# xp3i4/linear

Measured on AMD Instinct MI355X. Metric: reads/sec (whole node) + HBM GB/s on seed lookup, 10 kb reads vs GRCh38, higher is better.
Workload: dtype u64

## Files before the change

linear_amd/build.py:

```python
from __future__ import annotations

import os
import shutil
import subprocess

HERE = os.path.dirname(os.path.abspath(__file__))
CSRC = os.path.join(HERE, "csrc")
SO = os.path.join(HERE, "liblinear_amd.so")
CLI = os.path.join(HERE, "linear_filter")
SOURCES = sorted(f for f in os.listdir(CSRC) if f.endswith((".hip", ".h", ".cpp", ".inc")))
FLAGS = ["--offload-arch=gfx950", "-O3", "-std=c++17", "-ffp-contract=off", "-fPIC", "-shared"]


def hipcc_path() -> str:
    for c in (shutil.which("hipcc"), "/opt/rocm/bin/hipcc"):
        if c and os.path.exists(c):
            return c
    raise RuntimeError("hipcc not found: the MI355X library cannot be built")


def needs_build() -> bool:
    if not os.path.exists(SO) or not os.path.exists(CLI):
        return True
    t = os.path.getmtime(SO)
    deps = [os.path.join(CSRC, s) for s in SOURCES] + [os.path.join(HERE, "..", "include", "linear_amd.h")]
    return any(os.path.getmtime(d) > t for d in deps)


DEVICE_TUS = ["lnr_api.hip", "lnr_gap_kernels.hip", "lnr_output_kernels.hip", "lnr_reader_kernels.hip"]
OUT_GPU = {"lnr_output_kernels.hip", "lnr_output_hd.h", "lnr_output_hook.h", "lnr_deflate_hd.h", "lnr_inflate_hd.h"}
RD_GPU = {"lnr_reader_kernels.hip", "lnr_reader_hd.h", "lnr_reader_hook.h", "lnr_inflate_hd.h", "lnr_bam_hd.h"}
API_HOST = {"lnr_host_util.h", "lnr_ctx.h", "lnr_index.h", "lnr_batch.h", "lnr_gap_stage.h"}
NOT_A_DEP = {"lnr_api.hip": {"lnr_gap_kernels.hip", "lnr_gap_hd.h", "lnr_reader.cpp", "lnr_output.cpp", "linear_filter_main.cpp"} | OUT_GPU | RD_GPU,
             "lnr_gap_kernels.hip": {"lnr_api.hip", "lnr_kernels.hip", "lnr_reader.cpp", "lnr_output.cpp", "linear_filter_main.cpp"} | OUT_GPU | RD_GPU | API_HOST,
             "lnr_output_kernels.hip": set(SOURCES) - OUT_GPU - {"ref_sort.h"},
             "lnr_reader_kernels.hip": set(SOURCES) - RD_GPU,
             "lnr_reader.cpp": set(SOURCES) - {"lnr_reader.cpp", "lnr_reader_hook.h", "lnr_inflate_hd.h", "lnr_bam_hd.h"}, "lnr_output.cpp": set(SOURCES) - {"lnr_output.cpp", "lnr_output_hook.h"}}


def stale(obj: str, src: str) -> bool:
    if not os.path.exists(obj):
        return True
    t = os.path.getmtime(obj)
    deps = [os.path.join(CSRC, f) for f in SOURCES if f not in NOT_A_DEP[src]] + [os.path.join(HERE, "..", "include", "linear_amd.h"), os.path.abspath(__file__)]
    return any(os.path.getmtime(d) > t for d in deps)


def build(force: bool = False, defines: tuple = (), out: str | None = None, only: tuple | None = None) -> str:
    so = out or SO
    if out and only:
        build()
        tag = "." + os.path.basename(out).replace(".so", "")
        stock = [os.path.join(HERE, s.replace(".cpp", ".o")) for s in ("lnr_reader.cpp", "lnr_output.cpp")] + [os.path.join(HERE, s.replace(".hip", ".o")) for s in DEVICE_TUS if s not in only]
        mine = [(os.path.join(HERE, s.replace(".hip", tag + ".o")), s) for s in only]
        note, want = out + ".defines", " ".join(defines) + "\n"
        same = os.path.exists(note) and open(note).read() == want
        if not force and same and os.path.exists(out) and not any(stale(o, s) or os.path.getmtime(o) > os.path.getmtime(out) for o, s in mine) and all(os.path.getmtime(o) <= os.path.getmtime(out) for o in stock):
            return out
        for obj, src in mine:
            cmd = [hipcc_path()] + [f for f in FLAGS if f != "-shared"] + list(defines) + ["-c", os.path.join(CSRC, src), "-o", obj]
            if subprocess.call(cmd):
                raise RuntimeError("compile failed: " + " ".join(cmd))
        os.makedirs(os.path.dirname(out), exist_ok=True)
        subprocess.check_call([hipcc_path(), "--offload-arch=gfx950", "-fPIC", "-shared", "-o", out] + ["-Wl," + o for o in stock + [o for o, _ in mine]] + ["-lz", "-lpthread"])
        with open(note, "w") as f:
            f.write(want)
        return out
    if force or out or needs_build():
        from concurrent.futures import ThreadPoolExecutor
        tag = "" if not out else "." + os.path.basename(out).replace(".so", "")
        jobs = []
        for src in ("lnr_reader.cpp", "lnr_output.cpp"):
            obj = os.path.join(HERE, src.replace(".cpp", ".o"))
            jobs.append((obj, None if not (force or stale(obj, src)) else ["g++", "-O2", "-std=c++17", "-fPIC", "-Wall", "-Wextra", "-c", os.path.join(CSRC, src), "-o", obj]))
        for src in DEVICE_TUS:
            obj = os.path.join(HERE, src.replace(".hip", tag + ".o"))
            jobs.append((obj, None if not (force or out or stale(obj, src)) else
                         [hipcc_path()] + [f for f in FLAGS if f != "-shared"] + list(defines) + ["-c", os.path.join(CSRC, src), "-o", obj]))
        with ThreadPoolExecutor(len(jobs)) as ex:
            for rc, (obj, cmd) in zip(ex.map(lambda j: subprocess.call(j[1]) if j[1] else 0, jobs), jobs):
                if rc:
                    raise RuntimeError("compile failed: " + " ".join(cmd))
        objs = ["-Wl," + o for o, _ in jobs]
        subprocess.check_call([hipcc_path(), "--offload-arch=gfx950", "-fPIC", "-shared", "-o", so] + objs + ["-lz", "-lpthread"])
        if not out:
            subprocess.check_call(["g++", "-O2", "-std=c++17", "-Wall", "-Wextra", os.path.join(CSRC, "linear_filter_main.cpp"), "-o", CLI, SO,
                                   "-Wl,-rpath,$ORIGIN", "-Wl,-rpath,/opt/rocm/lib", "-L/opt/rocm/lib", "-lpthread"])
    return so


VARIANT_DIR = os.path.join(HERE, "..", "tools", "_variants")
GAP_VARIANTS = {
    "columns": ("-DK_GAP_COL_MIN=64", "-DK_GAP_COL_MEAN=1", "-DK_GAP_YB_MIN=64", "-DK_GAP_SORT_TEAM_MIN=128", "-DK_GAP_JOIN_TEAM_MIN=256"),
    "scan": ("-DK_GAP_COL_MIN=64", "-DK_GAP_COL_MEAN=1", "-DK_GAP_YB_MIN=1000000000", "-DK_GAP_SORT_TEAM_MIN=128", "-DK_GAP_JOIN_TEAM_MIN=256"),
    "rows": ("-DK_GAP_COL_MIN=1000000000", "-DK_GAP_TEAM_ROW=256", "-DK_GAP_SINGLE_MAX=1024", "-DK_GAP_SORT_TEAM_MIN=128", "-DK_GAP_JOIN_TEAM_MIN=256"),
}


def gap_variant_path(name: str) -> str:
    return os.path.abspath(os.path.join(VARIANT_DIR, "gap_" + name + ".so"))


def build_gap_variants() -> list:
    from concurrent.futures import ThreadPoolExecutor
    build()
    with ThreadPoolExecutor(len(GAP_VARIANTS)) as ex:
        return list(ex.map(lambda kv: build(defines=kv[1], out=gap_variant_path(kv[0]), only=("lnr_gap_kernels.hip",)), GAP_VARIANTS.items()))


if __name__ == "__main__":
    import sys
    if len(sys.argv) > 1:
        vdir = os.path.join(HERE, "..", "tools", "_variants")
        os.makedirs(vdir, exist_ok=True)
        print(build(defines=tuple(sys.argv[2:]), out=os.path.join(vdir, sys.argv[1] + ".so")))
    else:
        print(build(force=True))
```

linear_amd/csrc/lnr_api.hip:

```cpp
#include <cstring>
#include <rocprim/device/device_radix_sort.hpp>
#include "lnr_kernels.hip"
#include "lnr_gap_args.h"
#include "../../include/linear_amd.h"

#include <algorithm>
#include <dlfcn.h>
#include <chrono>
#include <cstdio>
#include <cstdlib>
#include <atomic>
#include <condition_variable>
#include <deque>
#include <memory>
#include <mutex>
#include <string>
#include <thread>
#include <vector>

using namespace lnr;

#include "lnr_host_util.h"
#include "lnr_ctx.h"
#include "lnr_index.h"
#include "lnr_batch.h"

namespace {

lnr_status submit_reads(lnr_ctx *ctx, Lane *L, int slot, const u8 *reads, const u64 *off, u32 n) {
    if (!off || (n && !reads)) { ctx->err = "null read buffer"; return LNR_ERR_ARG; }
    for (u32 i = 0; i < n; i++)
        if (off[i + 1] < off[i]) { ctx->err = "read offsets not monotone"; return LNR_ERR_ARG; }
    u64 base = off[0], total = off[n] - off[0];
    DevBuf &dr = L->in_reads[slot], &dof = L->in_off[slot];
    AllocCount count_(&L->allocs);
    ENSURE(dr, std::max<u64>(total, 16));
    ENSURE(dof, ((size_t)n + 1) * 8);
    if (!L->h_off[slot].ensure(((size_t)n + 1) * 8)) { ctx->err = "pinned host allocation failed"; return LNR_ERR_NOMEM; }
    u64 *o = L->h_off[slot].as<u64>();
    for (u32 i = 0; i <= n; i++) o[i] = off[i] - base;
    hipStream_t sc = ctx->s_copy;
    if (total) {
        hipPointerAttribute_t at;
        bool pinned = hipPointerGetAttributes(&at, reads + base) == hipSuccess && at.type == hipMemoryTypeHost;
        if (!pinned) (void)hipGetLastError();
        if (pinned) {
            HIPCK(hipMemcpyAsync(dr.p, reads + base, total, hipMemcpyHostToDevice, sc));
        } else {
            const u64 CH = 32ULL << 20;
            for (int k = 0; k < 2; k++) {
                if (!ctx->h_up[k].ensure(CH)) { ctx->err = "pinned host allocation failed"; return LNR_ERR_NOMEM; }
                HIPCK(ctx->ev_up[k].create());
            }
            int k = 0;
            for (u64 o2 = 0; o2 < total; o2 += CH, k ^= 1) {
                u64 len = std::min<u64>(CH, total - o2);
                HIPCK(hipEventSynchronize(ctx->ev_up[k]));
                par_memcpy(ctx->h_up[k].p, reads + base + o2, len);
                HIPCK(hipMemcpyAsync(dr.as<u8>() + o2, ctx->h_up[k].p, len, hipMemcpyHostToDevice, sc));
                HIPCK(hipEventRecord(ctx->ev_up[k], sc));
            }
        }
    }
    HIPCK(hipMemcpyAsync(dof.p, o, ((size_t)n + 1) * 8, hipMemcpyHostToDevice, sc));
    HIPCK(hipEventRecord(L->ev_in[slot], sc));
    L->in_n[slot] = n;
    return LNR_OK;
}

std::unique_ptr<Lane> lane_create(lnr_ctx *ctx, int id) {
    std::unique_ptr<Lane> L(new (std::nothrow) Lane());
    if (!L) return nullptr;
    L->opts = &ctx->opts; L->tun = &ctx->tun; L->ix = &ctx->ix; L->id = id;
    if (!L->init(id == 1 ? ctx->tun.lane1_prio : 0)) return nullptr;
    return L;
}

void lane_release_batch(Lane *L) {
    for (int k = 0; k < 2; k++) { L->js[k].anchors.release(); L->js[k].cap_slots = 0; }
    L->ln.job_scr.release(); L->tb_remap.scr.release(); L->tb_early.scr.release(); L->tb_late.scr.release();
    L->pk.release(); L->nm.release(); L->f1.release(); L->cords.release(); L->out_str.release(); L->out_end.release(); L->gaps.release(); L->gdense.release();
}

lnr_status compute_slot(Lane *C, Lane *In, int slot, Pre &P) {
    P = Pre();
    P.valid = true; P.tot = 0; P.n = In->in_n[slot];
    hipError_t e = hipStreamWaitEvent(C->stream, In->ev_in[slot], 0);
    P.st = e == hipSuccess ? filter_dev(C, In->in_reads[slot].as<u8>(), In->in_off[slot].as<u64>(), In->in_n[slot], nullptr, In->h_off[slot].as<u64>()) : LNR_ERR_HIP;
    P.err = C->err.get();
    P.stats = C->stats;
    if (P.st == LNR_OK) {
        P.tot = C->last_ncords;
        if (C->h_cord_off.size() != (size_t)P.n + 1) C->h_cord_off.assign((size_t)P.n + 1, 0);
        P.coff = C->h_cord_off;
        P.d_str = C->r_str.p; P.d_end = C->r_end.p;
    }
    return P.st;
}
lnr_status compute_submitted(lnr_ctx *ctx) {
    int slot = ctx->in_head;
    ctx->in_head = (ctx->in_head + 1) % 3; ctx->in_count--;
    return compute_slot(ctx->lane[0].get(), ctx->lane[0].get(), slot, ctx->pre);
}

void lane_worker(lnr_ctx *top, int li) {
    Lane &Ln = *top->lane[li], &L0 = *top->lane[0];
    (void)hipSetDevice(top->device);
    std::unique_lock<std::mutex> lk(top->mu);
    auto take_set = [](Lane &R, Ticket *T) {
        T->res_set = R.set_used[0] ? 1 : 0;
        R.set_used[T->res_set] = true;
    };
    auto run = [&](Lane &R, Ticket *T) {
        if (T->res_set != R.set_cur) { R.r_off.swap(R.rB_off); R.r_str.swap(R.rB_str); R.r_end.swap(R.rB_end); R.set_cur = T->res_set; }
        compute_slot(&R, &Ln, T->slot, T->pre);
        if (T->pre.st == LNR_OK && !R.rB_str.p) {
            AllocCount count_(&R.allocs);
            (void)R.rB_off.ensure(R.r_off.cap); (void)R.rB_off.host_stage(R.r_off.hcap); (void)R.rB_str.ensure(R.r_str.cap); (void)R.rB_end.ensure(R.r_end.cap);
        }
    };
    for (;;) {
        top->cv.wait(lk, [&] { return top->quit || (!Ln.work.empty() && (li == 1 || (Ln.unhanded < 2 && !Ln.busy && !(top->lane1_off && top->lane[1] && top->lane[1]->pending > 0))) && (li == 0 || top->lane1_off || Ln.unhanded < 2)); });
        if (top->quit) return;
        Ticket *T = Ln.work.front();
        Ln.work.pop_front();
        bool on_own = li == 0 || !top->lane1_off;
        if (on_own) {
            Ln.busy = true;
            take_set(Ln, T);
            lk.unlock();
            if (li == 1 && top->lane1_nomem_test) { top->lane1_nomem_test = false; T->pre = Pre(); T->pre.valid = true; T->pre.st = LNR_ERR_NOMEM; T->pre.err = "LNR_LANE1_NOMEM: allocation failure injected"; }
            else run(Ln, T);
            lk.lock();
            Ln.busy = false;
            if (li == 1 && T->pre.st == LNR_ERR_NOMEM) {
                Ln.set_used[T->res_set] = false;
                top->lane1_off = true;
                on_own = false;
                lk.unlock();
                Ln.sync();
                lane_release_batch(&Ln);
                if (getenv("LNR_DEBUG_TIMES")) fprintf(stderr, "[lnr] lane 1 out of memory: its batch runs again on lane 0, one lane from now on\n");
                lk.lock();
                top->cv.notify_all();
            }
        }
        if (!on_own) {
            top->cv.wait(lk, [&] { return top->quit || (!L0.busy && L0.unhanded < 2); });
            if (top->quit) return;
            L0.busy = true;
            take_set(L0, T);
            lk.unlock();
            run(L0, T);
            lk.lock();
            L0.busy = false;
        }
        Lane &R = on_own ? Ln : L0;
        T->res_lane = on_own ? li : 0;
        T->done = true;
        Ln.slot_busy[T->slot] = false; Ln.pending--; R.unhanded++;
        top->cv.notify_all();
    }
}

lnr_status hand_out(lnr_ctx *ctx, u32 n, u64 tot, std::vector<u64> &&coff, const void *d_str, const void *d_end, hipStream_t st, hipStream_t after, lnr_cords *out) {
    const int rs = ctx->res_slot;
    ctx->res_slot ^= 1;
    PinBuf &hs_ = ctx->h_cords_str2[rs], &he_ = ctx->h_cords_end2[rs];
    if (!hs_.ensure(std::max<u64>(tot * 8, 16)) || !he_.ensure(std::max<u64>(tot * 8, 16))) { ctx->err = "pinned host allocation failed"; return LNR_ERR_NOMEM; }
    ctx->h_cord_off2[rs] = std::move(coff);
    if (tot) {
        if (after) { HIPCK(hipEventRecord(ctx->ev_done, after)); HIPCK(hipStreamWaitEvent(st, ctx->ev_done, 0)); }
        HIPCK(hipMemcpyAsync(hs_.p, d_str, tot * 8, hipMemcpyDeviceToHost, st));
        HIPCK(hipMemcpyAsync(he_.p, d_end, tot * 8, hipMemcpyDeviceToHost, st));
    }
    out->n_reads = n; out->n_cords = tot;
    out->cord_off = ctx->h_cord_off2[rs].data(); out->cords_str = hs_.as<u64>(); out->cords_end = he_.as<u64>();
    return LNR_OK;
}

lnr_status lane0_result(lnr_ctx *ctx, lnr_status st) {
    if (st != LNR_OK) ctx->err = ctx->lane[0]->err.get();
    ctx->stats_pub = ctx->lane[0]->stats;
    return st;
}

}

extern "C" {

void lnr_opts_default(lnr_opts *o) {
    if (!o) return;
    memset(o, 0, sizeof *o);
    o->device = -1; o->index_type = 1; o->feature_type = 2; o->preset = 1; o->gap_len = 0; o->dup = 0; o->scratch_budget = 0;
}

const char *lnr_strerror(lnr_status s) {
    switch (s) {
        case LNR_OK: return "ok";
        case LNR_ERR_ARG: return "invalid argument";
        case LNR_ERR_NO_DEVICE: return "no usable HIP device (this library has no CPU path)";
        case LNR_ERR_HIP: return "HIP runtime error";
        case LNR_ERR_NOMEM: return "out of memory";
        case LNR_ERR_NO_INDEX: return "index not built";
        case LNR_ERR_LIMIT: return "input exceeds a format limit";
        case LNR_ERR_UNSUPPORTED: return "option not supported by this build";
        case LNR_ERR_INTERNAL: return "internal capacity overflow";
    }
    return "unknown status";
}
const char *lnr_last_error(const lnr_ctx *ctx) { return ctx ? const_cast<lnr_ctx *>(ctx)->err.show() : "null context"; }

lnr_status lnr_create(const lnr_opts *opts, lnr_ctx **out) {
    if (!out) return LNR_ERR_ARG;
    *out = nullptr;
    lnr_opts o;
    if (opts) o = *opts; else lnr_opts_default(&o);
    if ((o.index_type != 1 && o.index_type != 2) || o.feature_type != 2 || (o.preset != 1 && o.preset != 2) || o.dup > 1) return LNR_ERR_UNSUPPORTED;
    int ndev = 0;
    if (hipGetDeviceCount(&ndev) != hipSuccess || ndev <= 0) { (void)hipGetLastError(); return LNR_ERR_NO_DEVICE; }
    int dev = o.device;
    if (dev < 0) { if (hipGetDevice(&dev) != hipSuccess) return LNR_ERR_NO_DEVICE; }
    if (dev >= ndev) return LNR_ERR_ARG;
    int prev_dev = -1;
    (void)hipGetDevice(&prev_dev);
    if (hipSetDevice(dev) != hipSuccess) return LNR_ERR_NO_DEVICE;
    struct Restore { int d; ~Restore() { if (d >= 0) (void)hipSetDevice(d); } } restore_{prev_dev == dev ? -1 : prev_dev};
    lnr_ctx *ctx = new (std::nothrow) lnr_ctx();
    if (!ctx) return LNR_ERR_NOMEM;
    ctx->opts = o;
    ctx->device = dev;
    ctx->tun = tuning_from_env(dev);
    ctx->lane1_nomem_test = ctx->tun.lane1_nomem;
    ctx->lane[0] = lane_create(ctx, 0);
    bool ok = ctx->lane[0] && ctx->s_copy.create() && ctx->s_down.create() && ctx->ev_down.create() == hipSuccess && ctx->ev_done.create() == hipSuccess;
    if (!ok) { (void)hipGetLastError(); lnr_destroy(ctx); return LNR_ERR_HIP; }
    *out = ctx;
    return LNR_OK;
}

void lnr_destroy(lnr_ctx *ctx) {
    if (!ctx) return;
    (void)hipSetDevice(ctx->device);
    { std::lock_guard<std::mutex> g(ctx->mu); ctx->quit = true; }
    ctx->cv.notify_all();
    for (auto &L : ctx->lane) if (L && L->th.joinable()) L->th.join();
    ctx->s_copy.sync(); ctx->s_down.sync();
    delete ctx;
}

lnr_status lnr_filter_batch_dev(lnr_ctx *ctx, const uint8_t *d_reads, const uint64_t *d_off, uint32_t n, lnr_cords_dev *out) {
    if (!ctx || !d_off || (n && !d_reads)) return LNR_ERR_ARG;
    DevGuard dg_(ctx->device);
    if (in_flight(ctx)) { ctx->err = "batches submitted with lnr_filter_submit are still in flight"; return LNR_ERR_ARG; }
    return lane0_result(ctx, filter_dev(ctx->lane[0].get(), d_reads, d_off, n, out));
}
lnr_status lnr_last_gaps(lnr_ctx *ctx, lnr_gaps *out) {
    if (!ctx || !out) return LNR_ERR_ARG;
    DevGuard dg_(ctx->device);
    if (!ctx->tickets.empty()) { ctx->err = "lnr_last_gaps: batches are in flight (a worker is writing the per-read arrays)"; return LNR_ERR_ARG; }
    Lane *L = ctx->lane[0].get();
    u32 n = L->last_n;
    out->n_reads = n; out->n_gaps = 0; out->gap_off = nullptr; out->gaps = nullptr;
    ctx->h_gap_off.assign((size_t)n + 1, 0);
    ctx->h_gap_pairs.clear();
    if (n && L->last_gaps_off.size() == n) {
        std::vector<u32> ng(n);
        HIPCK(hipStreamSynchronize(L->stream));
        HIPCK(hipMemcpy(ng.data(), L->ngaps.p, (size_t)n * 4, hipMemcpyDeviceToHost));
        for (u32 i = 0; i < n; i++) ctx->h_gap_off[i + 1] = ctx->h_gap_off[i] + ng[i];
        ctx->h_gap_pairs.resize(2 * ctx->h_gap_off[n]);
        u64 last = L->last_gaps_off[n - 1];
        std::vector<UP> all;
        {
            u64 total_cap = last + 4 + (1u << 10);
            if (total_cap * sizeof(UP) > L->gaps.cap) total_cap = L->gaps.cap / sizeof(UP);
            all.resize(total_cap);
            if (total_cap) HIPCK(hipMemcpy(all.data(), L->gaps.p, total_cap * sizeof(UP), hipMemcpyDeviceToHost));
        }
        for (u32 i = 0; i < n; i++)
            for (u32 k = 0; k < ng[i]; k++) {
                const UP &g = all[L->last_gaps_off[i] + k];
                ctx->h_gap_pairs[2 * (ctx->h_gap_off[i] + k)] = g.first; ctx->h_gap_pairs[2 * (ctx->h_gap_off[i] + k) + 1] = g.second;
            }
    }
    out->n_gaps = ctx->h_gap_off[n];
    out->gap_off = ctx->h_gap_off.data(); out->gaps = ctx->h_gap_pairs.data();
    return LNR_OK;
}
lnr_status lnr_cords_to_host(lnr_ctx *ctx, lnr_cords *out) {
    if (!ctx || !out) return LNR_ERR_ARG;
    DevGuard dg_(ctx->device);
    if (!ctx->tickets.empty()) { ctx->err = "lnr_cords_to_host: batches are in flight"; return LNR_ERR_ARG; }
    Lane *L = ctx->lane[0].get();
    u64 tot = L->last_ncords;
    if (L->h_cord_off.size() != (size_t)L->last_n + 1) L->h_cord_off.assign((size_t)L->last_n + 1, 0);
    lnr_status s = hand_out(ctx, L->last_n, tot, std::vector<u64>(L->h_cord_off), L->r_str.p, L->r_end.p, L->stream, nullptr, out);
    if (s != LNR_OK) return s;
    if (tot) HIPCK(hipStreamSynchronize(L->stream));
    return LNR_OK;
}
void *lnr_host_alloc(size_t bytes) {
    void *p = nullptr;
    if (hipHostMalloc(&p, bytes ? bytes : 16, hipHostMallocDefault) != hipSuccess) { (void)hipGetLastError(); return nullptr; }
    return p;
}
void lnr_host_free(void *p) { if (p) (void)hipHostFree(p); }

lnr_status lnr_filter_submit(lnr_ctx *ctx, const uint8_t *reads, const uint64_t *off, uint32_t n) {
    if (!ctx) return LNR_ERR_ARG;
    DevGuard dg_(ctx->device);
    if (!ctx->ix.has_index) { ctx->err = "no index"; return LNR_ERR_NO_INDEX; }
    if (ctx->in_count + (ctx->pre.valid ? 1 : 0) + ctx->tickets.size() >= 3) { ctx->err = "three batches already in flight: call lnr_filter_wait first"; return LNR_ERR_ARG; }
    if (two_lanes(ctx)) {
        int li = (ctx->tickets.empty() || ctx->lane1_off) ? 0 : (ctx->tickets.back()->lane ^ 1);
        if (li == 1 && !ctx->lane[1]) {
            std::unique_ptr<Lane> L1 = lane_create(ctx, 1);
            if (L1) { std::lock_guard<std::mutex> g(ctx->mu); ctx->lane[1] = std::move(L1); }
            else { ctx->lane1_off = true; li = 0; }
        }
        int slot = 0;
        for (;;) {
            Lane &Ln = *ctx->lane[li];
            { std::lock_guard<std::mutex> g(ctx->mu); slot = 0; while (slot < 2 && Ln.slot_busy[slot]) slot++; }
            lnr_status s = submit_reads(ctx, &Ln, slot, reads, off, n);
            if (s == LNR_ERR_NOMEM && li == 1) { ctx->lane1_off = true; li = 0; continue; }
            if (s != LNR_OK) return s;
            break;
        }
        Lane &Ln = *ctx->lane[li];
        if (!Ln.th.joinable()) {
            try { Ln.th = std::thread(lane_worker, ctx, li); }
            catch (...) { ctx->err = "worker thread could not be started"; return LNR_ERR_INTERNAL; }
        }
        std::unique_ptr<Ticket> T(new Ticket());
        T->lane = li; T->slot = slot;
        {
            std::lock_guard<std::mutex> g(ctx->mu);
            Ln.slot_busy[slot] = true; Ln.pending++;
            Ln.work.push_back(T.get());
        }
        ctx->tickets.push_back(std::move(T));
        ctx->cv.notify_all();
        return LNR_OK;
    }
    int slot = (ctx->in_head + ctx->in_count) % 3;
    lnr_status s = submit_reads(ctx, ctx->lane[0].get(), slot, reads, off, n);
    if (s != LNR_OK) return s;
    ctx->in_count++;
    return LNR_OK;
}
lnr_status lnr_filter_wait(lnr_ctx *ctx, lnr_cords *out) {
    if (!ctx || !out) return LNR_ERR_ARG;
    DevGuard dg_(ctx->device);
    if (!ctx->tickets.empty()) {
        Ticket *T = ctx->tickets.front().get();
        { std::unique_lock<std::mutex> lk(ctx->mu); ctx->cv.wait(lk, [&] { return T->done; }); }
        Pre P = std::move(T->pre);
        Lane &Ln = *ctx->lane[T->res_lane];
        const int T_set = T->res_set;
        ctx->tickets.pop_front();
        struct Free { lnr_ctx *c; Lane &l; int set; ~Free() { { std::lock_guard<std::mutex> g(c->mu); l.unhanded--; l.set_used[set] = false; } c->cv.notify_all(); } } free_{ctx, Ln, T_set};
        if (P.st != LNR_OK) { ctx->err = P.err; return P.st; }
        lnr_status s = hand_out(ctx, P.n, P.tot, std::move(P.coff), P.d_str, P.d_end, ctx->s_down, nullptr, out);
        if (s != LNR_OK) return s;
        if (P.tot) HIPCK(hipStreamSynchronize(ctx->s_down));
        ctx->stats_pub = P.stats;
        return LNR_OK;
    }
    if (!ctx->pre.valid) {
        if (ctx->in_count == 0) { ctx->err = "no batch in flight"; return LNR_ERR_ARG; }
        compute_submitted(ctx);
    }
    Pre P = std::move(ctx->pre);
    ctx->pre = Pre();
    if (P.st != LNR_OK) { ctx->err = P.err; return P.st; }
// ... 83 lines not shown
```

linear_amd/csrc/lnr_batch.h:

```cpp
#pragma once
#include "lnr_gap_stage.h"

namespace {

struct HostJobs {
    std::vector<u32> read, str, end, mode, grp_beg;
    u64 nsamp = 0;
    void add(u32 r, u32 s, u32 e, u32 m) {
        read.push_back(r); str.push_back(s); end.push_back(e); mode.push_back(m);
        nsamp += seed_num_samples(s, e, (u32)job_parm((int)m).alpha);
    }
    u32 size() const { return (u32)read.size(); }
};

struct BatchHost {
    u32 n = 0;
    std::vector<u64> off;
    std::vector<u32> len, nf, cords_cap, gaps_cap;
    std::vector<u64> f1_off, cords_off, gaps_off, pk_off;
};

JobArrays job_arrays(JobSet &S) {
    JobArrays J;
    J.read = S.j_read.as<u32>(); J.str = S.j_str.as<u32>(); J.end = S.j_end.as<u32>(); J.mode = S.j_mode.as<u32>();
    return J;
}
ReadArrays read_arrays(Lane *L) {
    ReadArrays R;
    R.len = L->rlen.as<u32>(); R.ks = L->rks.as<i32>();
    R.pk = L->pk.as<u64>(); R.nm = L->nm.as<u32>(); R.pk_off = L->pk_off.as<u64>();
    return R;
}

lnr_status launch_f1(Lane *L, u32 n) {
    LCK(hipEventRecord(L->ev_prep, L->stream));
    LCK(hipStreamWaitEvent(L->s_bulk, L->ev_prep, 0));
    hipLaunchKernelGGL(k_f1, dim3(n), dim3(256), 0, L->s_bulk, L->pk.as<u64>(), L->nm.as<u32>(), L->pk_off.as<u64>(), L->rlen.as<u32>(), L->nf.as<u32>(), L->f1_off.as<u64>(), n,
                       L->f1.as<F96>()); LKCHECK();
    LCK(hipEventRecord(L->ev_f1, L->s_bulk));
    return LNR_OK;
}

lnr_status seed_jobs(Lane *L, JobSet &S, const HostJobs &hj, hipStream_t st, u32 f1_reads = 0) {
    const Index &ix = *L->ix; const Tuning &tun = *L->tun;
    u32 nj = hj.size();
    S.cap.assign(nj, 0); S.look.assign(nj, 0); S.nanc.assign(nj, 0); S.anc_off.assign(nj, 0);
    if (nj == 0) return f1_reads ? launch_f1(L, f1_reads) : LNR_OK;
    lnr_status s;
    if ((s = upload_on(L->err, S.j_read, hj.read, st)) != LNR_OK) return s;
    if ((s = upload_on(L->err, S.j_str, hj.str, st)) != LNR_OK) return s;
    if ((s = upload_on(L->err, S.j_end, hj.end, st)) != LNR_OK) return s;
    if ((s = upload_on(L->err, S.j_mode, hj.mode, st)) != LNR_OK) return s;
    if ((s = upload_on(L->err, S.grp_beg, hj.grp_beg, st)) != LNR_OK) return s;
    LENSURE(S.j_cap, (size_t)nj * 4);
    LENSURE(S.j_look, (size_t)nj * 4);
    LENSURE(S.j_nanc, (size_t)nj * 4);
    LENSURE(S.j_anc_off, (size_t)nj * 8);
    LENSURE(S.seed_ctl, 64);
    if (!S.t_seed.a) S.t_seed.init();
    JobArrays J = job_arrays(S);
    ReadArrays R = read_arrays(L);
    u64 first_segs = ((hj.nsamp * S.est_x16) >> 4) + (u64)nj * 194;
    u64 need_slots = first_segs * 2 + (1u << 20);
    if (need_slots > S.cap_slots) S.cap_slots = need_slots + need_slots / 2;
    u64 anc_slots = S.cap_slots;
    bool use_bm = tun.seed_bm < 0 ? ix.info.hs_len < (1ULL << 25) : tun.seed_bm != 0;
    for (int attempt = 0; ; attempt++) {
        LENSURE(S.anchors, anc_slots * 8);
        LCK(hipMemsetAsync(S.seed_ctl.p, 0, 64, st));
        SeedOutArrays O;
        O.cursor = S.seed_ctl.as<unsigned long long>(); O.overflow = (int *)(S.seed_ctl.as<char>() + 16); O.capacity = anc_slots;
        O.anchors = S.anchors.as<u64>(); O.anc_off = S.j_anc_off.as<u64>(); O.job_cap = S.j_cap.as<u32>(); O.job_look = S.j_look.as<u32>();
        O.n_anchors = S.j_nanc.as<u32>();
        S.t_seed.start(st);
        if (L->opts->index_type == 2)
            hipLaunchKernelGGL(k_seed_hindex, dim3(nj), dim3(64), 0, st, J, R, ix.hs.as<u64>(), ix.info.hs_len, ix.hx_empty_dir, ix.dir.as<i32>(), ix.hx_nkeys.as<u64>(), ix.hx_nvals.as<u32>(), ix.hx_nnodes, nj, O,
                               S.est_x16);
        else
        hipLaunchKernelGGL(k_seed_fused, dim3(nj), dim3(64), tun.seed_lds_pad, st, J, R, ix.bl.as<ulonglong2>(), use_bm ? ix.bm.as<u32>() : (const u32 *)nullptr, ix.ov.as<u64>(), nj, O, S.est_x16); LKCHECK();
        S.t_seed.stop(st);
        if (f1_reads && attempt == 0) { lnr_status fs = launch_f1(L, f1_reads); if (fs != LNR_OK) return fs; }
        int ovf = 0;
        Readback rb;
        if (!rb.begin(S.h_rb, (size_t)nj * 20 + 256)) { L->err = "pinned host allocation failed"; return LNR_ERR_NOMEM; }
        LCK(rb.add(S.cap.data(), S.j_cap.p, (size_t)nj * 4, st));
        LCK(rb.add(S.look.data(), S.j_look.p, (size_t)nj * 4, st));
        LCK(rb.add(S.nanc.data(), S.j_nanc.p, (size_t)nj * 4, st));
        LCK(rb.add(S.anc_off.data(), S.j_anc_off.p, (size_t)nj * 8, st));
        LCK(rb.add(&ovf, S.seed_ctl.as<char>() + 16, 4, st));
        LCK(hipStreamSynchronize(st));
        rb.finish();
        if (!ovf) {
            L->stats.seed_count_ms += S.t_seed.ms();
            L->stats.seed_count_launches++;
            break;
        }
        if (attempt == 5) { L->err = "anchor buffer overflow after five resizes"; return LNR_ERR_INTERNAL; }
        anc_slots *= 2;
        S.cap_slots = anc_slots;
    }
    {
        u64 tot = 0;
        for (u32 j = 0; j < nj; j++) tot += S.nanc[j];
        if (hj.nsamp) {
            S.est_x16 = (u32)std::min<u64>(std::max<u64>((tot * 24) / hj.nsamp + 8, 32), 400 * 16);
        }
    }
    L->stats.jobs += nj;
    L->stats.samples += hj.nsamp;
    for (u32 j = 0; j < nj; j++) { L->stats.lookups += S.look[j]; L->stats.bucket_entries += S.cap[j] - 1; L->stats.anchors += S.nanc[j] - 1; }
    return LNR_OK;
}

lnr_status export_anchors(Lane *L, JobSet &S, u32 nj, std::vector<u64> &a_off, std::vector<u64> &a_vals) {
    a_off.assign((size_t)nj + 1, 0);
    for (u32 j = 0; j < nj; j++) a_off[j + 1] = a_off[j] + S.nanc[j];
    a_vals.resize(a_off[nj]);
    u64 used = 0;
    for (u32 j = 0; j < nj; j++) used = std::max<u64>(used, S.anc_off[j] + S.nanc[j]);
    std::vector<u64> all(used);
    if (used) LCK(hipMemcpy(all.data(), S.anchors.p, used * 8, hipMemcpyDeviceToHost));
    for (u32 j = 0; j < nj; j++) memcpy(a_vals.data() + a_off[j], all.data() + S.anc_off[j], (size_t)S.nanc[j] * 8);
    return LNR_OK;
}

lnr_status launch_jobs(Lane *L, JobSet &S, const HostJobs &hj) {
    const Index &ix = *L->ix; const Tuning &tun = *L->tun;
    u32 ngrp = (u32)hj.grp_beg.size() - 1;
    if (ngrp == 0) return LNR_OK;
    Laps laps;
    u32 nj = hj.size();
    Launch &Lx = L->ln;
    hipStream_t sm = L->stream, sb = L->s_bulk;
    u64 budget = L->opts->scratch_budget ? L->opts->scratch_budget : (64ULL << 30);
    const std::vector<u32> &nanc = S.nanc;
    std::vector<u64> w(ngrp, 0);
    for (u32 k = 0; k < ngrp; k++) for (u32 j = hj.grp_beg[k]; j < hj.grp_beg[k + 1]; j++) w[k] += nanc[j];
    std::vector<u32> order(ngrp);
    {
        auto cls = [](u64 v) -> u32 {
            if (v < 8) return (u32)v;
            int lg = 63 - __builtin_clzll(v);
            return (u32)(8 * (lg - 2) + ((v >> (lg - 3)) & 7));
        };
        const u32 NCLS = 8 * 64;
        std::vector<u32> cnt(NCLS + 1, 0), gc(ngrp);
        for (u32 k = 0; k < ngrp; k++) { gc[k] = NCLS - 1 - std::min<u32>(cls(w[k]), NCLS - 1); cnt[gc[k] + 1]++; }
        for (u32 c = 0; c < NCLS; c++) cnt[c + 1] += cnt[c];
        for (u32 k = 0; k < ngrp; k++) order[cnt[gc[k]]++] = k;
        u32 nh = 0;
        while (nh < ngrp && w[order[nh]] >= std::min(std::min(tun.heavy_cap, tun.mid_cap), std::min(tun.heavy_cap_r1, tun.mid_cap_r1)) / 2) nh++;
        if (nh <= 4096) std::stable_sort(order.begin(), order.begin() + nh, [&w](u32 a, u32 b) { return w[a] > w[b]; });
    }
    Lx.h_order = order;
    laps.lap("order");
    lnr_status s;
    if ((s = upload_on(L->err, Lx.grp_order, Lx.h_order, sm)) != LNR_OK) return s;
    laps.lap("upload-order");
    LENSURE(Lx.j_scr_off, (size_t)nj * 8);
    std::vector<u64> &scr_off = Lx.h_scr_off;
    scr_off.assign(nj, 0);
    auto grp_scr = [&](u32 g) { u64 b = 0; for (u32 j = hj.grp_beg[g]; j < hj.grp_beg[g + 1]; j++) b += align_up(job_scratch_bytes((u64)nanc[j] + 2), 256); return b; };
    u32 g0 = 0;
    while (g0 < ngrp) {
        u64 scr = 0;
        u32 g1 = g0;
        while (g1 < ngrp) {
            u64 s2 = scr + grp_scr(order[g1]);
            if (g1 > g0 && s2 > budget) break;
            scr = s2; g1++;
        }
        u64 so = 0;
        for (u32 k = g0; k < g1; k++)
            for (u32 j = hj.grp_beg[order[k]]; j < hj.grp_beg[order[k] + 1]; j++) { scr_off[j] = so; so += align_up(job_scratch_bytes((u64)nanc[j] + 2), 256); }
        laps.lap("scr-layout");
        LENSURE(Lx.job_scr, std::max<u64>(so, 16));
        laps.lap("ensure-scr");
        {
            void *h = Lx.j_scr_off.host_stage((size_t)nj * 8);
            if (!h) { L->err = "pinned host allocation failed"; return LNR_ERR_NOMEM; }
            memcpy(h, scr_off.data(), (size_t)nj * 8);
            LCK(words_in(Lx.j_scr_off.p, h, (size_t)nj * 8, sm));
        }
        laps.lap("upload-scr");
        JobArgs A;
        A.grp_order = Lx.grp_order.as<u32>(); A.grp_beg = S.grp_beg.as<u32>(); A.J = job_arrays(S);
        A.anc_off = S.j_anc_off.as<u64>(); A.job_cap = S.j_cap.as<u32>(); A.n_anchors = S.j_nanc.as<u32>(); A.scr_off = Lx.j_scr_off.as<u64>();
        A.anchors = S.anchors.as<u64>(); A.scratch = Lx.job_scr.as<char>();
        A.read_len = L->rlen.as<u32>(); A.f1_off = L->f1_off.as<u64>(); A.nf = L->nf.as<u32>(); A.f1 = L->f1.as<F96>();
        A.g.base = ix.f2.as<F96>(); A.g.off = ix.d_f2_off.as<u64>(); A.g.nseq = ix.info.nseq;
        A.cords = L->cords.as<u64>(); A.cords_off = L->cords_off.as<u64>(); A.cords_cap = L->cords_cap.as<u32>(); A.ncords = L->ncords.as<u32>();
        A.read_err = L->read_err.as<i32>();
        A.nbins = ix.nbins; A.grp_lo = g0; A.grp_hi = g1;
        A.prof = nullptr; A.tl = nullptr; A.stop_after = tun.stop_after;
        size_t lds = (tun.job_lds_bytes + 15) & ~(size_t)15;
        A.lds_bytes = (u32)lds;
        A.arena_lds = (u32)lds;
        bool remap_round_ = nj && hj.mode[0] != 0;
        u64 hcap = remap_round_ ? tun.heavy_cap_r1 : tun.heavy_cap, mcap = remap_round_ ? tun.mid_cap_r1 : tun.mid_cap;
        if (!remap_round_ && !tun.mid_cap_env && ix.info.hs_len >= (1ULL << 25)) mcap = 9000;
        u32 gh = g0;
        while (gh < g1 && w[order[gh]] >= hcap) gh++;
        u32 gm = gh;
        while (gm < g1 && w[order[gm]] >= mcap) gm++;
#ifdef LNR_PROF
        if (!L->prof.p) { if (!L->prof.ensure(192 * 8)) return LNR_ERR_NOMEM; (void)hipMemsetAsync(L->prof.p, 0, 192 * 8, sm); }
        A.prof = L->prof.as<unsigned long long>();
        if (!L->tl.p) { if (!L->tl.ensure(4ULL * (1u << 20) * 32)) return LNR_ERR_NOMEM; (void)hipMemsetAsync(L->tl.p, 0, 4ULL * (1u << 20) * 32, sm); }
        if (L->tl_round < 4 && g1 <= (1u << 20)) { A.tl = L->tl.as<unsigned long long>() + (size_t)L->tl_round * (1u << 20) * 4; L->tl_n[L->tl_round] = g1; L->tl_nh[L->tl_round] = gm; }
        L->tl_round++;
#endif
        hipStream_t smid = gh > g0 ? L->s_spare : sm;
        bool fork_m = gm > gh && gh > g0, fork_b = g1 > gm && gm > g0;
        if (fork_m || fork_b) LCK(hipEventRecord(L->ev_fork, sm));
        if (gh > g0) {
            JobArgs H = A;
            size_t hl = (size_t)tun.heavy_lds_kb * 1024;
            H.grp_lo = g0; H.grp_hi = gh; H.lds_bytes = (u32)hl; H.arena_lds = (u32)hl;
            hipLaunchKernelGGL(k_job_heavy, dim3(gh - g0), dim3(1024), hl, sm, H); LKCHECK();
        }
        if (gm > gh) {
            if (fork_m) LCK(hipStreamWaitEvent(smid, L->ev_fork, 0));
            JobArgs M = A;
            size_t ml = (size_t)tun.mid_lds_kb * 1024;
            M.grp_lo = gh; M.grp_hi = gm; M.lds_bytes = (u32)ml; M.arena_lds = (u32)ml;
            if (tun.mid_waves == 2 || (tun.mid_waves == 0 && !remap_round_ && ix.info.hs_len >= (1ULL << 25)))
                hipLaunchKernelGGL(k_job_mid2, dim3(gm - gh), dim3(128), ml, smid, M);
            else hipLaunchKernelGGL(k_job_mid, dim3(gm - gh), dim3(256), ml, smid, M); LKCHECK();
            if (fork_m) LCK(hipEventRecord(L->ev_join_spare, smid));
        }
        if (g1 > gm) {
            hipStream_t bulk = fork_b ? sb : sm;
            if (fork_b) {
                LCK(hipStreamWaitEvent(sb, L->ev_fork, 0));
                hipLaunchKernelGGL(k_delay, dim3(1), dim3(64), 0, sb, tun.bulk_delay_ticks); LKCHECK();
            }
            JobArgs K = A;
            K.grp_lo = gm; K.grp_hi = g1;
            hipLaunchKernelGGL(k_job, dim3(g1 - gm), dim3(64), lds, bulk, K); LKCHECK();
        }
        if (fork_b) { LCK(hipEventRecord(L->ev_join_bulk, sb)); LCK(hipStreamWaitEvent(sm, L->ev_join_bulk, 0)); }
        if (fork_m) LCK(hipStreamWaitEvent(sm, L->ev_join_spare, 0));
        laps.lap("launches");
        L->stats.job_launches++;
        g0 = g1;
        if (g0 < ngrp) LCK(hipStreamSynchronize(sm));
    }
    if (laps.on && std::chrono::duration<double, std::milli>(std::chrono::steady_clock::now() - laps.t0).count() > 1.5) laps.done();
    return LNR_OK;
}

lnr_status prepare_batch(Lane *L, const u8 *d_reads, const u64 *d_off, u32 n, BatchHost &B, const u64 *h_off = nullptr) {
    const Tuning &tun = *L->tun;
    B.n = n;
    B.off.resize((size_t)n + 1);
    if (h_off) memcpy(B.off.data(), h_off, ((size_t)n + 1) * 8);
    else {
        Readback rb;
        if (!rb.begin(L->h_rb[0], ((size_t)n + 1) * 8)) { L->err = "pinned host allocation failed"; return LNR_ERR_NOMEM; }
        LCK(rb.add(B.off.data(), d_off, ((size_t)n + 1) * 8, L->stream));
        LCK(hipStreamSynchronize(L->stream));
        rb.finish();
    }
    B.len.resize(n); B.nf.resize(n); B.cords_cap.resize(n); B.gaps_cap.resize(n);
    B.f1_off.resize(n); B.cords_off.resize(n); B.gaps_off.resize(n); B.pk_off.resize(n);
    u64 fo = 0, co = 0, go = 0, po = 0;
    for (u32 i = 0; i < n; i++) {
        if (B.off[i + 1] < B.off[i]) { L->err = "read offsets not monotone"; return LNR_ERR_ARG; }
        u64 len = B.off[i + 1] - B.off[i];
        if (len >= (1ULL << 20)) { L->err = "read longer than 2^20-1 bases (cord y field, cords.cpp:15)"; return LNR_ERR_LIMIT; }
        B.len[i] = (u32)len;
        B.pk_off[i] = po; po += 2 * packed_words(len);
        B.nf[i] = len > 200 ? read_feature_count(len) : 0;
        B.f1_off[i] = fo; fo += 2ULL * B.nf[i];
        B.cords_cap[i] = len > 200 ? (u32)std::min<u64>(std::max<u64>((16 * (len / 64) + 256) / tun.cap_shrink, 8) * L->cap_scale, 1u << 24) : 0;
        B.cords_off[i] = co; co += B.cords_cap[i];
        B.gaps_cap[i] = len > 200 ? (u32)((len / 1000 + 4) * L->cap_scale) : 0;
        B.gaps_off[i] = go; go += B.gaps_cap[i];
    }
    lnr_status s;
    if ((s = upload_on(L->err, L->rlen, B.len, L->stream)) != LNR_OK) return s;
    if ((s = upload_on(L->err, L->pk_off, B.pk_off, L->stream)) != LNR_OK) return s;
    LENSURE(L->pk, std::max<u64>(po * 8, 16));
    LENSURE(L->nm, std::max<u64>(po * 4, 16));
    if ((s = upload_on(L->err, L->nf, B.nf, L->stream)) != LNR_OK) return s;
    if ((s = upload_on(L->err, L->f1_off, B.f1_off, L->stream)) != LNR_OK) return s;
    if ((s = upload_on(L->err, L->cords_cap, B.cords_cap, L->stream)) != LNR_OK) return s;
    if ((s = upload_on(L->err, L->cords_off, B.cords_off, L->stream)) != LNR_OK) return s;
    if ((s = upload_on(L->err, L->gaps_cap, B.gaps_cap, L->stream)) != LNR_OK) return s;
    if ((s = upload_on(L->err, L->gaps_off, B.gaps_off, L->stream)) != LNR_OK) return s;
    LENSURE(L->rks, (size_t)n * 4);
    LENSURE(L->f1, std::max<u64>(fo * sizeof(F96), 16));
    LENSURE(L->cords, std::max<u64>(co * 8, 16));
    LENSURE(L->out_str, std::max<u64>(co * 8, 16));
    LENSURE(L->out_end, std::max<u64>(co * 8, 16));
    LENSURE(L->gaps, std::max<u64>(go * sizeof(UP), 16));
    LENSURE(L->gdense, std::max<u64>(go * sizeof(UP), 16));
    LENSURE(L->gcursor, 16);
    LENSURE(L->gpos, (size_t)n * 4);
    LENSURE(L->ncords, (size_t)n * 4);
    LENSURE(L->nout, (size_t)n * 4);
    LENSURE(L->read_err, (size_t)n * 4);
    LENSURE(L->ngaps, (size_t)n * 4);
    LENSURE(L->remap, (size_t)n * 4);
    LCK(hipMemsetAsync(L->ncords.p, 0, (size_t)n * 4, L->stream));
    LCK(hipMemsetAsync(L->read_err.p, 0, (size_t)n * 4, L->stream));
    L->t_prep.start(L->stream);
    hipLaunchKernelGGL(k_prep, dim3(n < tun.prep_grid ? n : tun.prep_grid), dim3(tun.prep_threads), 0, L->stream, d_reads, d_off, L->pk_off.as<u64>(), n, L->pk.as<u64>(), L->nm.as<u32>(), L->rks.as<i32>()); LKCHECK();
    L->t_prep.stop(L->stream);
    L->stats.reads = n;
    L->stats.bases = B.off[n] - B.off[0];
    return LNR_OK;
}

lnr_status tail_prepare(Lane *L, const BatchHost &B, TailBuf &tb, const std::vector<u32> *list, hipStream_t st, TailArgs &T) {
    u32 n = B.n;
    std::vector<u32> ncords(n);
    {
        Readback rb;
        PinBuf &pb = L->h_rb[st == L->s_tail ? 2 : 1];
        if (!rb.begin(pb, (size_t)n * 4)) { L->err = "pinned host allocation failed"; return LNR_ERR_NOMEM; }
        LCK(rb.add(ncords.data(), L->ncords.p, (size_t)n * 4, st));
        LCK(hipStreamSynchronize(st));
        rb.finish();
    }
    tb.h_off.assign(n, 0); tb.h_cap.assign(n, 0);
    u64 o = 0;
    u32 cnt = list ? (u32)list->size() : n;
    for (u32 k = 0; k < cnt; k++) {
        u32 i = list ? (*list)[k] : k;
        tb.h_cap[i] = ncords[i] + 4; tb.h_off[i] = o; o += align_up(tail_scratch_bytes(tb.h_cap[i]), 256);
    }
    lnr_status s;
    if ((s = upload_on(L->err, tb.off, tb.h_off, st)) != LNR_OK) return s;
    if ((s = upload_on(L->err, tb.cap, tb.h_cap, st)) != LNR_OK) return s;
    LENSURE(tb.scr, std::max<u64>(o, 16));
    T.read_len = L->rlen.as<u32>(); T.n = cnt; T.list = nullptr;
    if (list) {
        tb.h_list = *list;
        if ((s = upload_on(L->err, tb.list, tb.h_list, st)) != LNR_OK) return s;
        T.list = tb.list.as<u32>();
    }
    T.cords = L->cords.as<u64>(); T.cords_off = L->cords_off.as<u64>(); T.cords_cap = L->cords_cap.as<u32>(); T.ncords = L->ncords.as<u32>();
    T.read_err = L->read_err.as<i32>();
    T.scratch = tb.scr.as<char>(); T.scr_off = tb.off.as<u64>(); T.scr_cap = tb.cap.as<u32>();
    T.gaps = L->gaps.as<UP>(); T.gaps_off = L->gaps_off.as<u64>(); T.gaps_cap = L->gaps_cap.as<u32>(); T.ngaps = L->ngaps.as<u32>(); T.remap = L->remap.as<u32>();
    T.gdense = L->gdense.as<UP>(); T.gcursor = L->gcursor.as<u32>(); T.gpos = L->gpos.as<u32>();
    T.out_str = L->out_str.as<u64>(); T.out_end = L->out_end.as<u64>(); T.nout = L->nout.as<u32>();
    return LNR_OK;
}

void reset_stats(Lane *L) { memset(&L->stats, 0, sizeof L->stats); }
void finish_stats(Lane *L, const BatchHost &B) {
    u64 rb = 0;
    for (u32 i = 0; i < B.n; i++) if (B.len[i] > 200) rb += (B.len[i] + 3) / 4;
    L->stats.seed_bytes = rb + L->stats.lookups * 8 + L->stats.bucket_entries * 8 + L->stats.anchors * 8;
}

lnr_status remap_round(Lane *L, const BatchHost &B, HostJobs &j1) {
    hipStream_t st = L->stream;
    JobSet &S = L->js[1];
    u32 n = B.n;
    TailArgs T;
    lnr_status s;
    if ((s = tail_prepare(L, B, L->tb_remap, nullptr, st, T)) != LNR_OK) return s;
    Laps laps;
    laps.lap("tail_prepare");
    LCK(hipMemsetAsync(L->gcursor.p, 0, 4, st));
    hipLaunchKernelGGL(k_tail_a, dim3((T.n + 63) / 64), dim3(64), 0, st, T); LKCHECK();
    if (!L->h_flags.ensure((size_t)n * 12 + 16)) { L->err = "pinned host allocation failed"; return LNR_ERR_NOMEM; }
    u32 *remap = L->h_flags.as<u32>(), *ngaps = remap + n, *gpos = ngaps + n, *gtot_p = gpos + n;
    LCK(copy_words(remap, L->remap.p, n, st));
    LCK(copy_words(ngaps, L->ngaps.p, n, st));
    LCK(copy_words(gpos, L->gpos.p, n, st));
    LCK(copy_words(gtot_p, L->gcursor.p, 1, st));
    LCK(hipStreamSynchronize(st));
    laps.lap("tail_a+flags");
    u64 gtot = *gtot_p;
    if (gtot == 0) return LNR_OK;
    if (!L->h_gaps.ensure(gtot * sizeof(UP))) { L->err = "pinned host allocation failed"; return LNR_ERR_NOMEM; }
    UP *gaps = L->h_gaps.as<UP>();
    LCK(copy_words(gaps, L->gdense.p, gtot * sizeof(UP) / 4, st));
    LCK(hipStreamSynchronize(st));
    for (u32 i = 0; i < n; i++) {
        if (!(remap[i] && ngaps[i])) continue;
        L->stats.remap_reads++;
        j1.grp_beg.push_back(j1.size());
        for (u32 k = 0; k < ngaps[i]; k++) {
            UP y = forward_y(gaps[gpos[i] + k], B.len[i]);
            j1.add(i, (u32)y.first, (u32)y.second, 1);
        }
    }
    j1.grp_beg.push_back(j1.size());
    laps.lap("gaps-copy+build");
    if ((s = seed_jobs(L, S, j1, st)) != LNR_OK) return s;
    laps.lap("seed1(sync)");
    s = launch_jobs(L, S, j1);
    laps.lap("launch1");
    laps.done();
    return s;
}

lnr_status filter_dev(Lane *L, const u8 *d_reads, const u64 *d_off, u32 n, lnr_cords_dev *out, const u64 *h_off = nullptr, int attempt = 0) {
    const Index &ix = *L->ix;
    if (!ix.has_index) { L->err = "no index: call lnr_index_build or lnr_index_adopt first"; return LNR_ERR_NO_INDEX; }
    reset_stats(L);
    AllocCount count_(&L->allocs);
    L->last_n = n; L->last_ncords = 0;
    if (out) { out->n_reads = n; out->n_cords = 0; out->d_cord_off = nullptr; out->d_cords_str = nullptr; out->d_cords_end = nullptr; }
    LENSURE(L->r_off, ((size_t)n + 1) * 8);
    if (n == 0) {
        LCK(hipMemsetAsync(L->r_off.p, 0, 8, L->stream));
        LCK(hipStreamSynchronize(L->stream));
        if (out) out->d_cord_off = L->r_off.as<u64>();
        return LNR_OK;
    }
    Laps laps;
    L->t_total.start(L->stream);
    BatchHost B;
    lnr_status s = prepare_batch(L, d_reads, d_off, n, B, h_off);
    if (s != LNR_OK) return s;
    L->last_gaps_off = B.gaps_off;
    laps.lap("prepare");
    HostJobs j0;
    for (u32 i = 0; i < n; i++) {
        if (B.len[i] > 200) { j0.grp_beg.push_back(j0.size()); j0.add(i, 0, B.len[i], 0); }
    }
    j0.grp_beg.push_back(j0.size());
    if ((s = seed_jobs(L, L->js[0], j0, L->stream, n)) != LNR_OK) return s;
    laps.lap("seed0(sync)");
    LCK(hipStreamWaitEvent(L->stream, L->ev_f1, 0));
    L->t_job.start(L->stream);
    LCK(hipEventRecord(L->ev_start, L->stream));
    LCK(hipStreamWaitEvent(L->s_spare, L->ev_start, 0));
    LCK(hipStreamWaitEvent(L->s_bulk, L->ev_start, 0));
    laps.lap("events");
    if ((s = launch_jobs(L, L->js[0], j0)) != LNR_OK) return s;
    laps.lap("launch0");
    LCK(hipStreamSynchronize(L->stream));
    HostJobs j1;
    if ((s = remap_round(L, B, j1)) != LNR_OK) return s;
    laps.lap("tailA+seed1+launch1");
    std::vector<u32> late_list, early_list;
    bool early = j1.size() > 0;
    if (early) {
        std::vector<char> in_r1(n, 0);
        for (u32 q = 0; q < j1.size(); q++) in_r1[j1.read[q]] = 1;
        for (u32 i = 0; i < n; i++) (in_r1[i] ? late_list : early_list).push_back(i);
        TailArgs TE;
        if ((s = tail_prepare(L, B, L->tb_early, &early_list, L->s_tail, TE)) != LNR_OK) return s;
        if (TE.n) { hipLaunchKernelGGL(k_tail_b, dim3((TE.n + 63) / 64), dim3(64), 0, L->s_tail, TE); LKCHECK(); }
        LCK(hipEventRecord(L->ev_prep, L->s_tail));
    }
    L->t_job.stop(L->stream);
    LCK(hipStreamSynchronize(L->stream));
    L->stats.job_ms += L->t_job.ms();
    laps.lap("wait-r1");
    TailArgs T;
    if ((s = tail_prepare(L, B, L->tb_late, early ? &late_list : nullptr, L->stream, T)) != LNR_OK) return s;
    L->t_tail.start(L->stream);
    if (T.n) { hipLaunchKernelGGL(k_tail_b, dim3((T.n + 63) / 64), dim3(64), 0, L->stream, T); LKCHECK(); }
    L->t_tail.stop(L->stream);
    if (early) LCK(hipStreamWaitEvent(L->stream, L->ev_prep, 0));
    int ext_state_out = L->gap_ext;
    if (L->opts->gap_len) {
        u32 maxlen = 0;
        for (u32 i = 0; i < n; i++) maxlen = std::max(maxlen, B.len[i]);
        if ((s = gap_stage(L, d_reads, d_off, n, maxlen, &ext_state_out)) != LNR_OK) return s;
    }
    std::vector<u32> nout(n);
    std::vector<i32> rerr(n);
    u32 gap_second = 0, gap_last = 0;
    {
        Readback rb;
        if (!rb.begin(L->h_rb[0], (size_t)n * 8 + 256)) { L->err = "pinned host allocation failed"; return LNR_ERR_NOMEM; }
        LCK(rb.add(nout.data(), L->nout.p, (size_t)n * 4, L->stream));
        LCK(rb.add(rerr.data(), L->read_err.p, (size_t)n * 4, L->stream));
        if (L->opts->gap_len) LCK(rb.add(&gap_second, L->gap_next.as<u32>() + 16, 4, L->stream));
        if (L->opts->gap_len) LCK(rb.add(&gap_last, L->gap_next.as<u32>() + 24 + 8, 4, L->stream));
        LCK(hipStreamSynchronize(L->stream));
        rb.finish();
    }
    L->stats.tail_ms += L->t_tail.ms();
    if (L->opts->gap_len) { L->stats.gap_ms += L->t_gap.ms(); L->stats.gap_second_pass += gap_second; L->stats.gap_last_launch += gap_last; }
    for (u32 i = 0; i < n; i++)
        if (rerr[i]) {
            if (attempt < 2) {
                L->t_total.stop(L->stream);
                LCK(hipStreamSynchronize(L->stream));
                L->cap_scale = attempt == 0 ? 4 : 16;
                L->overflow_reruns++;
                lnr_status rs = filter_dev(L, d_reads, d_off, n, out, h_off, attempt + 1);
                L->cap_scale = 1;
                return rs;
            }
            char b[160];
            snprintf(b, sizeof b, "device capacity overflow on read %u (stage code %d, length %u) with 16x capacities", i, rerr[i], B.len[i]);
            L->err = b;
            return LNR_ERR_INTERNAL;
        }
    L->gap_ext = ext_state_out;
    L->h_cord_off.assign((size_t)n + 1, 0);
    for (u32 i = 0; i < n; i++) L->h_cord_off[i + 1] = L->h_cord_off[i] + nout[i];
    u64 tot = L->h_cord_off[n];
    LENSURE(L->r_str, std::max<u64>(tot * 8, 16));
    LENSURE(L->r_end, std::max<u64>(tot * 8, 16));
    {
        void *h = L->r_off.host_stage(((size_t)n + 1) * 8);
        if (!h) { L->err = "pinned host allocation failed"; return LNR_ERR_NOMEM; }
        memcpy(h, L->h_cord_off.data(), ((size_t)n + 1) * 8);
        LCK(words_in(L->r_off.p, h, ((size_t)n + 1) * 8, L->stream));
    }
    hipLaunchKernelGGL(k_gather_out, dim3(n), dim3(64), 0, L->stream, L->out_str.as<u64>(), L->out_end.as<u64>(), L->cords_off.as<u64>(), L->nout.as<u32>(),
                       L->r_off.as<u64>(), n, L->r_str.as<u64>(), L->r_end.as<u64>()); LKCHECK();
    L->t_total.stop(L->stream);
    LCK(hipStreamSynchronize(L->stream));
    laps.lap("tailB+gather");
    if (laps.on) { char b[64]; snprintf(b, sizeof b, " | lane %d allocations so far %u", L->id, L->allocs.load()); laps.out += b; }
    laps.done();
    L->stats.prep_ms = L->t_prep.ms();
    L->stats.total_ms = L->t_total.ms();
    L->stats.cords = tot;
    finish_stats(L, B);
    L->last_ncords = tot;
    if (out) { out->n_cords = tot; out->d_cord_off = L->r_off.as<u64>(); out->d_cords_str = L->r_str.as<u64>(); out->d_cords_end = L->r_end.as<u64>(); }
    return LNR_OK;
}

lnr_status seed_dev(Lane *L, const u8 *d_reads, const u64 *d_off, u32 n, bool to_host, std::vector<u64> &a_off, std::vector<u64> &a_vals) {
    const Index &ix = *L->ix;
    if (!ix.has_index) { L->err = "no index: call lnr_index_build or lnr_index_adopt first"; return LNR_ERR_NO_INDEX; }
    reset_stats(L);
    a_off.assign((size_t)n + 1, 0);
    a_vals.clear();
    if (n == 0) return LNR_OK;
    L->t_total.start(L->stream);
    BatchHost B;
    lnr_status s = prepare_batch(L, d_reads, d_off, n, B);
    if (s != LNR_OK) return s;
    HostJobs j0;
    std::vector<u32> job_of(n, 0xffffffffu);
    for (u32 i = 0; i < n; i++) {
        if (B.len[i] >= 43) { job_of[i] = j0.size(); j0.grp_beg.push_back(j0.size()); j0.add(i, 0, B.len[i], 0); }
    }
    j0.grp_beg.push_back(j0.size());
    if ((s = seed_jobs(L, L->js[0], j0, L->stream, n)) != LNR_OK) return s;
    if (to_host && (s = export_anchors(L, L->js[0], j0.size(), a_off, a_vals)) != LNR_OK) return s;
    LCK(hipStreamWaitEvent(L->stream, L->ev_f1, 0));
    L->t_total.stop(L->stream);
    LCK(hipStreamSynchronize(L->stream));
    L->stats.prep_ms = L->t_prep.ms();
    L->stats.total_ms = L->t_total.ms();
    u64 rb = 0;
    for (u32 i = 0; i < n; i++) if (job_of[i] != 0xffffffffu) rb += (B.len[i] + 3) / 4;
    L->stats.seed_bytes = rb + L->stats.lookups * 8 + L->stats.bucket_entries * 8 + L->stats.anchors * 8;
    if (to_host) {
        std::vector<u64> off((size_t)n + 1, 0), vals;
        for (u32 i = 0; i < n; i++) {
            u64 c = job_of[i] == 0xffffffffu ? 1 : a_off[job_of[i] + 1] - a_off[job_of[i]];
            off[i + 1] = off[i] + c;
        }
        vals.assign(off[n], 0);
        for (u32 i = 0; i < n; i++)
            if (job_of[i] != 0xffffffffu) {
                u64 a = a_off[job_of[i]], c = a_off[job_of[i] + 1] - a;
                memcpy(vals.data() + off[i], a_vals.data() + a, c * 8);
            }
        a_off.swap(off);
        a_vals.swap(vals);
    }
    return LNR_OK;
}

}
```

linear_amd/csrc/lnr_ctx.h:

```cpp
#pragma once

namespace {

struct Index {
    bool has_index = false;
    lnr_index_info info{};
    std::vector<u64> seq_len, seq_off, f2_off;
    u32 nbins = 0;
    DevBuf g, dir, hs, f2, d_seq_off, d_f2_off, d_seq_len;
    DevBuf bm, bl, ov;
    DevBuf hx_nkeys, hx_nvals; u32 hx_nnodes = 0; u64 hx_empty_dir = 0;
};

struct Tuning {
    size_t job_lds_bytes = 6 * 1024;
    u32 heavy_lds_kb = 48;
    u32 mid_cap = 6144, mid_lds_kb = 24;
    u32 heavy_cap = 0xffffffffu;
    u32 heavy_cap_r1 = 7000, mid_cap_r1 = 3000;
    u32 stop_after = 0;
    u32 mid_waves = 0;
    bool mid_cap_env = false;
    int seed_bm = -1;
    u32 prep_threads = 256;
    u32 prep_grid = 4096;
    u32 bulk_delay_ticks = 10000;
    u32 cap_shrink = 1;
    u32 seed_lds_pad = 0;
    u32 gap_arena2_mb = 64;
    u32 gap_teams = 96, ncu = 0;
    u32 gap_heavy_w = 60000;
    u64 gap_work_cap = 3000000;
    u32 nlanes = 2;
    int lane1_prio = 1;
    bool lane1_nomem = false;
};

Tuning tuning_from_env(int device) {
    Tuning t;
    if (const char *e = getenv("LNR_LANES")) { long v = atol(e); if (v == 1 || v == 2) t.nlanes = (u32)v; }
    if (const char *e = getenv("LNR_LANE1_NOMEM")) t.lane1_nomem = atoi(e) != 0;
    if (const char *e = getenv("LNR_LANE1_PRIO")) { long v = atol(e); if (v >= -1 && v <= 1) t.lane1_prio = (int)v; }
    if (const char *e = getenv("LNR_CAP_SHRINK")) { long v = atol(e); if (v >= 1 && v <= 4096) t.cap_shrink = (u32)v; }
    if (const char *e = getenv("LNR_GAP_TEAMS")) { long v = atol(e); if (v >= 1 && v <= 4096) t.gap_teams = (u32)v; }
    { hipDeviceProp_t pr; if (hipGetDeviceProperties(&pr, device) == hipSuccess) t.ncu = (u32)pr.multiProcessorCount; else (void)hipGetLastError(); }
    if (const char *e = getenv("LNR_GAP_HEAVY_W")) { long v = atol(e); if (v >= 1) t.gap_heavy_w = (u32)v; }
    if (const char *e = getenv("LNR_GAP_ARENA2_MB")) { long v = atol(e); if (v >= 1 && v <= 1024) t.gap_arena2_mb = (u32)v; }
    if (const char *e = getenv("LNR_GAP_WORK_CAP")) { long long v = atoll(e); if (v >= 0) t.gap_work_cap = (u64)v; }
    if (const char *e = getenv("LNR_SEED_LDS_PAD")) { long v = atol(e); if (v >= 0 && v <= 100000) t.seed_lds_pad = (u32)v; }
    if (const char *e = getenv("LNR_JOB_LDS_KB")) { long kb = atol(e); if (kb >= 1 && kb <= 156) t.job_lds_bytes = (size_t)kb * 1024; }
    if (const char *e = getenv("LNR_HEAVY_CAP")) { long v = atol(e); if (v >= 64) { t.heavy_cap = (u32)std::min<long>(v, 0xffffffffL); t.heavy_cap_r1 = t.heavy_cap; } }
    if (const char *e = getenv("LNR_HEAVY_LDS_KB")) { long v = atol(e); if (v >= 1 && v <= 56) t.heavy_lds_kb = (u32)v; }
    if (const char *e = getenv("LNR_MID_CAP")) { long v = atol(e); if (v >= 64) { t.mid_cap_env = true; t.mid_cap = (u32)std::min<long>(v, 0xffffffffL); t.mid_cap_r1 = t.mid_cap; } }
    if (const char *e = getenv("LNR_MID_LDS_KB")) { long v = atol(e); if (v >= 1 && v <= 56) t.mid_lds_kb = (u32)v; }
    if (const char *e = getenv("LNR_HEAVY_CAP_R1")) { long v = atol(e); if (v >= 64) t.heavy_cap_r1 = (u32)std::min<long>(v, 0xffffffffL); }
    if (const char *e = getenv("LNR_MID_CAP_R1")) { long v = atol(e); if (v >= 64) t.mid_cap_r1 = (u32)std::min<long>(v, 0xffffffffL); }
    if (const char *e = getenv("LNR_MID_WAVES")) t.mid_waves = atoi(e) == 2 ? 2 : 4;
    if (const char *e = getenv("LNR_SEED_BM")) t.seed_bm = atoi(e) ? 1 : 0;
    if (const char *e = getenv("LNR_STOP_AFTER")) { long v = atol(e); if (v >= 0 && v < 16) t.stop_after = (u32)v; }
    if (const char *e = getenv("LNR_PREP_GRID")) { long v = atol(e); if (v > 0) t.prep_grid = (u32)v; }
    if (const char *e = getenv("LNR_PREP_THREADS")) { long v = atol(e); if (v == 64 || v == 128 || v == 256) t.prep_threads = (u32)v; }
    if (const char *e = getenv("LNR_BULK_DELAY_US")) { long v = atol(e); if (v >= 0 && v <= 5000) t.bulk_delay_ticks = (u32)v * 100; }
    return t;
}

struct JobSet {
    DevBuf j_read, j_str, j_end, j_mode, j_cap, j_look, j_anc_off, j_nanc, grp_beg, anchors, seed_ctl;
    std::vector<u32> cap, look, nanc;
    std::vector<u64> anc_off;
    u32 est_x16 = 64;
    u64 cap_slots = 0;
    Timer t_seed;
    PinBuf h_rb;
};
struct Launch { DevBuf grp_order, j_scr_off, job_scr; std::vector<u32> h_order; std::vector<u64> h_scr_off; };
struct TailBuf { DevBuf off, cap, scr, list; std::vector<u64> h_off; std::vector<u32> h_cap, h_list; };

struct Pre { bool valid = false; lnr_status st = LNR_OK; u32 n = 0; u64 tot = 0; lnr_stats stats; std::vector<u64> coff; const void *d_str = nullptr, *d_end = nullptr; std::string err; };
struct Ticket { int lane = 0, slot = 0, res_lane = 0, res_set = 0; bool done = false; Pre pre; };

struct Lane {
    const lnr_opts *opts = nullptr;
    const Tuning *tun = nullptr;
    const Index *ix = nullptr;
    int id = 0;
    ErrText err;
    Stream stream, s_spare, s_bulk, s_tail;
    Event ev_fork, ev_join_spare, ev_join_bulk, ev_start, ev_prep, ev_f1;
    DevBuf in_reads[3], in_off[3];
    PinBuf h_off[3];
    Event ev_in[3];
    u32 in_n[3] = {0, 0, 0};
    DevBuf rlen, rks, nf, f1_off, f1, pk, nm, pk_off;
    DevBuf cords, out_str, out_end, cords_off, cords_cap, ncords, nout, read_err;
    DevBuf gaps, gaps_off, gaps_cap, ngaps, remap, gdense, gcursor, gpos;
    PinBuf h_gaps, h_flags;
    JobSet js[2];
    Launch ln;
    TailBuf tb_remap, tb_early, tb_late;
    PinBuf h_rb[3];
    DevBuf prof, tl; u32 tl_round = 0, tl_n[4] = {0, 0, 0, 0}; u32 tl_nh[4] = {0, 0, 0, 0};
    DevBuf gap_arena, gap_flag, gap_next, gap_prof, gap_first, gap_list, gap_rank, gap_weight;
    int gap_ext = 0;
    DevBuf r_off, r_str, r_end, rB_off, rB_str, rB_end;
    std::vector<u64> h_cord_off;
    std::vector<u64> last_gaps_off;
    u32 last_n = 0;
    u64 last_ncords = 0;
    u32 cap_scale = 1;
    u32 overflow_reruns = 0;
    lnr_stats stats{};
    Timer t_prep, t_job, t_tail, t_total, t_gap;
    std::atomic<unsigned> allocs{0};
    std::thread th;
    std::deque<Ticket *> work;
    bool slot_busy[3] = {false, false, false};
    u32 pending = 0;
    u32 unhanded = 0;
    bool busy = false;
    bool set_used[2] = {false, false};
    int set_cur = 0;

    bool init(int stream_prio) {
        bool ok = stream.create(stream_prio) && s_spare.create(stream_prio) && s_bulk.create(stream_prio) && s_tail.create(stream_prio);
        for (Event *e : {&ev_fork, &ev_join_spare, &ev_join_bulk, &ev_start, &ev_prep, &ev_f1, &ev_in[0], &ev_in[1], &ev_in[2]}) ok = ok && e->create() == hipSuccess;
        if (!ok) { (void)hipGetLastError(); return false; }
        t_prep.init(); t_job.init(); t_tail.init(); t_total.init(); t_gap.init();
        return true;
    }
    void sync() const { stream.sync(); s_spare.sync(); s_bulk.sync(); s_tail.sync(); }
    ~Lane() { sync(); }
};

}

struct lnr_ctx {
    lnr_opts opts;
    int device = 0;
    ErrText err;
    Index ix;
    Tuning tun;
    Stream s_copy, s_down;
    Event ev_down, ev_done;
    PinBuf h_up[2]; Event ev_up[2];
    PinBuf h_cords_str2[2], h_cords_end2[2];
    std::vector<u64> h_cord_off2[2]; int res_slot = 0;
    std::vector<u64> h_anchor_off, h_anchors, h_gap_off, h_gap_pairs;
    lnr_stats stats_pub{};
    Pre pre;
    int in_head = 0, in_count = 0;
    std::deque<std::unique_ptr<Ticket>> tickets;
    std::mutex mu;
    std::condition_variable cv;
    bool quit = false;
    std::atomic<bool> lane1_off{false};
    bool lane1_nomem_test = false;
    std::unique_ptr<Lane> lane[2];

    hipStream_t stream() const { return lane[0]->stream; }
};

namespace {
bool in_flight(const lnr_ctx *ctx) { return ctx->in_count || ctx->pre.valid || !ctx->tickets.empty(); }
bool two_lanes(const lnr_ctx *ctx) { return ctx->tun.nlanes == 2 && ctx->opts.gap_len == 0; }
}
```

linear_amd/csrc/lnr_host_util.h:

```cpp
#pragma once

namespace {

thread_local std::atomic<unsigned> *t_allocs = nullptr;
struct AllocCount {
    std::atomic<unsigned> *prev;
    explicit AllocCount(std::atomic<unsigned> *c) : prev(t_allocs) { t_allocs = c; }
    ~AllocCount() { t_allocs = prev; }
};

struct NoCopy { NoCopy() = default; NoCopy(const NoCopy &) = delete; NoCopy &operator=(const NoCopy &) = delete; };

struct DevBuf : NoCopy {
    void *p = nullptr;
    size_t cap = 0;
    bool ensure(size_t bytes) {
        if (bytes <= cap && p) return true;
        if (t_allocs) ++*t_allocs;
        bool grown = p != nullptr;
        if (p) { (void)hipFree(p); p = nullptr; cap = 0; }
        size_t nc = bytes + (grown ? bytes / 2 : bytes / 8) + 4096;
        if (hipMalloc(&p, nc) != hipSuccess) { p = nullptr; cap = 0; (void)hipGetLastError(); return false; }
        cap = nc;
        return true;
    }
    void *hp = nullptr;
    size_t hcap = 0;
    void *host_stage(size_t bytes) {
        if (bytes <= hcap && hp) return hp;
        if (t_allocs) ++*t_allocs;
        if (hp) { (void)hipHostFree(hp); hp = nullptr; hcap = 0; }
        size_t nc = bytes + bytes / 8 + 4096;
        if (hipHostMalloc(&hp, nc, hipHostMallocDefault) != hipSuccess) { hp = nullptr; hcap = 0; (void)hipGetLastError(); return nullptr; }
        hcap = nc;
        return hp;
    }
    void release() { if (p) (void)hipFree(p); p = nullptr; cap = 0; if (hp) (void)hipHostFree(hp); hp = nullptr; hcap = 0; }
    ~DevBuf() { release(); }
    template <class T> T *as() const { return (T *)p; }
    void swap(DevBuf &o) { std::swap(p, o.p); std::swap(cap, o.cap); std::swap(hp, o.hp); std::swap(hcap, o.hcap); }
};

struct PinBuf : NoCopy {
    void *p = nullptr;
    size_t cap = 0;
    bool ensure(size_t bytes) {
        if (bytes <= cap && p) return true;
        bool grown = p != nullptr;
        if (t_allocs) ++*t_allocs;
        if (p) { (void)hipHostFree(p); p = nullptr; cap = 0; }
        size_t nc = bytes + (grown ? bytes / 2 : bytes / 8) + 4096;
        if (hipHostMalloc(&p, nc, hipHostMallocDefault) != hipSuccess) { p = nullptr; cap = 0; (void)hipGetLastError(); return false; }
        cap = nc;
        return true;
    }
    ~PinBuf() { if (p) (void)hipHostFree(p); }
    template <class T> T *as() const { return (T *)p; }
};

struct Stream : NoCopy {
    hipStream_t s = nullptr;
    bool create(int prio = 0) {
        hipError_t e = prio ? hipStreamCreateWithPriority(&s, hipStreamNonBlocking, prio) : hipStreamCreateWithFlags(&s, hipStreamNonBlocking);
        if (e != hipSuccess) { s = nullptr; (void)hipGetLastError(); }
        return e == hipSuccess;
    }
    void sync() const { if (s) (void)hipStreamSynchronize(s); }
    ~Stream() { if (s) { (void)hipStreamSynchronize(s); (void)hipStreamDestroy(s); } }
    operator hipStream_t() const { return s; }
};
struct Event : NoCopy {
    hipEvent_t e = nullptr;
    hipError_t create() { hipError_t r = e ? hipSuccess : hipEventCreateWithFlags(&e, hipEventDisableTiming); if (r != hipSuccess) e = nullptr; return r; }
    ~Event() { if (e) (void)hipEventDestroy(e); }
    operator hipEvent_t() const { return e; }
};
struct Timer : NoCopy {
    hipEvent_t a = nullptr, b = nullptr;
    void init() { if (!a) (void)hipEventCreate(&a); if (!b) (void)hipEventCreate(&b); }
    ~Timer() { if (a) (void)hipEventDestroy(a); if (b) (void)hipEventDestroy(b); }
    void start(hipStream_t s) { (void)hipEventRecord(a, s); }
    void stop(hipStream_t s) { (void)hipEventRecord(b, s); }
    double ms() { float f = 0; if (hipEventSynchronize(b) != hipSuccess) return 0; (void)hipEventElapsedTime(&f, a, b); return f; }
};

static inline hipError_t copy_words(void *dst, const void *src, u64 nw, hipStream_t st) {
    if (!nw) return hipSuccess;
    hipLaunchKernelGGL(lnr::k_words_out, dim3((u32)std::min<u64>((nw + 255) / 256, 1024)), dim3(256), 0, st, (const u32 *)src, (u32 *)dst, nw);
    return hipGetLastError();
}

struct Readback {
    struct Item { void *dst; size_t off, bytes; };
    PinBuf *pin = nullptr;
    std::vector<Item> items;
    size_t used = 0;
    bool begin(PinBuf &p, size_t total) { pin = &p; items.clear(); used = 0; return p.ensure(total + 64 * 8); }
    hipError_t add(void *dst, const void *dsrc, size_t bytes, hipStream_t st) {
        size_t o = (used + 15) & ~(size_t)15;
        used = o + bytes;
        items.push_back({dst, o, bytes});
        return copy_words((char *)pin->p + o, dsrc, bytes / 4, st);
    }
    void finish() { for (auto &i : items) if (i.bytes) memcpy(i.dst, (char *)pin->p + i.off, i.bytes); }
};

static inline hipError_t words_in(void *d_dst, const void *h_pinned, size_t bytes, hipStream_t st) { return copy_words(d_dst, h_pinned, (bytes + 3) / 4, st); }

static const u64 SEQ_PAD = 64;
static inline u64 align_up(u64 v, u64 a) { return (v + a - 1) / a * a; }

struct ErrText {
    std::mutex m;
    std::string s, shown;
    ErrText &operator=(const std::string &v) { std::lock_guard<std::mutex> g(m); s = v; return *this; }
    ErrText &operator=(const char *v) { std::lock_guard<std::mutex> g(m); s = v; return *this; }
    std::string get() { std::lock_guard<std::mutex> g(m); return s; }
    const char *show() { std::lock_guard<std::mutex> g(m); shown = s; return shown.c_str(); }
};

#define HIPCK_TO(err, call) do { hipError_t e_ = (call); if (e_ != hipSuccess) { char b_[256]; snprintf(b_, sizeof b_, "%s failed: %s (%s:%d)", #call, hipGetErrorString(e_), __FILE__, __LINE__); \
                                 (err) = b_; (void)hipGetLastError(); return LNR_ERR_HIP; } } while (0)
#define ENSURE_TO(err, buf, bytes) do { if (!(buf).ensure(bytes)) { char b_[160]; snprintf(b_, sizeof b_, "device allocation of %zu bytes failed (%s:%d)", (size_t)(bytes), __FILE__, __LINE__); \
                                        (err) = b_; return LNR_ERR_NOMEM; } } while (0)
#define HIPCK(call) HIPCK_TO(ctx->err, call)
#define ENSURE(buf, bytes) ENSURE_TO(ctx->err, buf, bytes)
#define KCHECK() HIPCK(hipGetLastError())
#define LCK(call) HIPCK_TO(L->err, call)
#define LENSURE(buf, bytes) ENSURE_TO(L->err, buf, bytes)
#define LKCHECK() LCK(hipGetLastError())
#define HIPCK_CTX(c, call) do { hipError_t e__ = (call); if (e__ != hipSuccess) { (c)->err = std::string(#call) + ": " + hipGetErrorString(e__); return LNR_ERR_HIP; } } while (0)

template <class T>
lnr_status upload_on(ErrText &err, DevBuf &b, const std::vector<T> &v, hipStream_t st) {
    ENSURE_TO(err, b, std::max<size_t>(v.size() * sizeof(T), 16));
    if (!v.empty()) {
        void *h = b.host_stage(v.size() * sizeof(T));
        if (!h) { err = "pinned host allocation failed"; return LNR_ERR_NOMEM; }
        memcpy(h, v.data(), v.size() * sizeof(T));
        HIPCK_TO(err, words_in(b.p, h, v.size() * sizeof(T), st));
    }
    return LNR_OK;
}

struct Laps {
    bool on; std::chrono::steady_clock::time_point t0, t; std::string out;
    Laps() : on(getenv("LNR_DEBUG_TIMES") != nullptr) { t0 = t = std::chrono::steady_clock::now(); }
    void lap(const char *name) {
        if (!on) return;
        auto n = std::chrono::steady_clock::now();
        char b[96]; snprintf(b, sizeof b, " %s %.2f", name, std::chrono::duration<double, std::milli>(n - t).count());
        out += b; t = n;
    }
    void done() { if (on) fprintf(stderr, "[lnr] host laps (ms):%s | total %.2f\n", out.c_str(), std::chrono::duration<double, std::milli>(std::chrono::steady_clock::now() - t0).count()); }
};

void par_memcpy(void *dst, const void *src, size_t len) {
    const size_t MIN = 4u << 20;
    unsigned T = (unsigned)std::min<size_t>(4, len / MIN);
    if (T < 2) { memcpy(dst, src, len); return; }
    std::vector<std::thread> th;
    size_t per = ((len + T - 1) / T + 63) & ~(size_t)63;
    for (unsigned t = 1; t < T; t++) {
        size_t o = (size_t)t * per, l = o < len ? std::min(per, len - o) : 0;
        if (l) th.emplace_back([=]() { memcpy((char *)dst + o, (const char *)src + o, l); });
    }
    memcpy(dst, src, std::min(per, len));
    for (auto &t : th) t.join();
}

struct DevGuard {
    int prev = -1;
    explicit DevGuard(int dev) { if (hipGetDevice(&prev) != hipSuccess) prev = -1; if (prev != dev) (void)hipSetDevice(dev); else prev = -1; }
    ~DevGuard() { if (prev >= 0) (void)hipSetDevice(prev); }
};

}
```

linear_amd/csrc/lnr_kernels.hip:

```cpp
#pragma once
#include <hip/hip_runtime.h>
#include "lnr_hd.h"

namespace lnr {

}
#include "lnr_wave.h"
namespace lnr {

__global__ void __launch_bounds__(256) k_words_out(const u32 *src, u32 *dst, u64 n) {
    for (u64 i = (u64)blockIdx.x * blockDim.x + threadIdx.x; i < n; i += (u64)gridDim.x * blockDim.x) dst[i] = src[i];
}

#if defined(K_JOB_WAVES) && K_JOB_WAVES > 4
#define JOB_INLINE __forceinline__
#else
#define JOB_INLINE
#endif
#define SCAN_TPB 256
#define SCAN_IPT 16
#define SCAN_BLK (SCAN_TPB * SCAN_IPT)

__global__ void __launch_bounds__(SCAN_TPB) k_scan_blk(const i32 *in, i32 *out, u64 n, i32 *blk_sums) {
    __shared__ i32 sh[SCAN_TPB];
    u64 base = (u64)blockIdx.x * SCAN_BLK + (u64)threadIdx.x * SCAN_IPT;
    i32 v[SCAN_IPT];
    i32 sum = 0;
#pragma unroll
    for (int k = 0; k < SCAN_IPT; k++) { u64 idx = base + k; v[k] = idx < n ? in[idx] : 0; sum += v[k]; }
    sh[threadIdx.x] = sum;
    __syncthreads();
    for (int off = 1; off < SCAN_TPB; off <<= 1) {
        i32 t = threadIdx.x >= (unsigned)off ? sh[threadIdx.x - off] : 0;
        __syncthreads();
        sh[threadIdx.x] += t;
        __syncthreads();
    }
    i32 run = sh[threadIdx.x] - sum;
    if (threadIdx.x == SCAN_TPB - 1) blk_sums[blockIdx.x] = sh[SCAN_TPB - 1];
#pragma unroll
    for (int k = 0; k < SCAN_IPT; k++) { u64 idx = base + k; if (idx < n) out[idx] = run; run += v[k]; }
}
__global__ void __launch_bounds__(1024) k_scan_top(i32 *blk, u32 nblk) {
    __shared__ i32 sh[1024];
    __shared__ i32 carry;
    if (threadIdx.x == 0) carry = 0;
    __syncthreads();
    for (u32 base = 0; base < nblk; base += 1024) {
        u32 i = base + threadIdx.x;
        i32 v = i < nblk ? blk[i] : 0;
        sh[threadIdx.x] = v;
        __syncthreads();
        for (int off = 1; off < 1024; off <<= 1) {
            i32 t = threadIdx.x >= (unsigned)off ? sh[threadIdx.x - off] : 0;
            __syncthreads();
            sh[threadIdx.x] += t;
            __syncthreads();
        }
        i32 c = carry;
        if (i < nblk) blk[i] = c + sh[threadIdx.x] - v;
        __syncthreads();
        if (threadIdx.x == 1023) carry = c + sh[1023];
        __syncthreads();
    }
}
__global__ void __launch_bounds__(SCAN_TPB) k_scan_add(i32 *out, u64 n, const i32 *blk) {
    u64 base = (u64)blockIdx.x * SCAN_BLK + (u64)threadIdx.x * SCAN_IPT;
    i32 add = blk[blockIdx.x];
#pragma unroll
    for (int k = 0; k < SCAN_IPT; k++) { u64 idx = base + k; if (idx < n) out[idx] += add; }
}

__global__ void __launch_bounds__(256) k_clamp_bases(u8 *g, u64 n16) {
    u64 i = (u64)blockIdx.x * blockDim.x + threadIdx.x;
    if (i >= n16) return;
    uint4 v = ((uint4 *)g)[i];
    u32 w[4] = {v.x, v.y, v.z, v.w};
    bool ch = false;
#pragma unroll
    for (int k = 0; k < 4; k++) {
        u32 x = w[k], hi = x & 0xF8F8F8F8u, c5 = ((x & 0x07070707u) + 0x03030303u) & 0x08080808u;
        u32 bad = ((hi | (hi >> 1) | (hi >> 2) | (hi >> 3) | (hi >> 4)) & 0x08080808u) | c5;
        if (bad) { u32 m = (bad >> 3) * 0xFFu; w[k] = (x & ~m) | (0x04040404u & m); ch = true; }
    }
    if (ch) ((uint4 *)g)[i] = make_uint4(w[0], w[1], w[2], w[3]);
}
struct ChunkDesc { u64 seq_off; i64 t_str; u64 samp_base; u32 nsamp; u32 seq_id; i32 ks; i32 C; };
static const u32 X_MASK = (1u << 26) - 1, X_REC = 1u << 30, X_FIRST = 1u << 31;

__global__ void __launch_bounds__(256) k_ix_chunk_const(const u8 *g, u64 gbytes, ChunkDesc *ch, u32 nch) {
    __shared__ unsigned long long s_best;
    u32 c = blockIdx.x;
    if (c >= nch) return;
    u64 s0 = ch[c].seq_off + (u64)ch[c].t_str;
    u64 found = ~0ULL;
    for (u64 tile = 0;; tile += 256 * 64) {
        if (threadIdx.x == 0) s_best = ~0ULL;
        __syncthreads();
        u64 seg = tile + (u64)threadIdx.x * 64;
        int run = 0;
        u64 mine = ~0ULL;
        for (int q = 0; q < 64 + 20; q++) {
            u64 idx = s0 + seg + (u64)q;
            if ((idx < gbytes ? g[idx] : (u8)0) == 4) run = 0; else run++;
            if (run >= 21 && q - 20 >= 0 && q - 20 < 64) { mine = seg + (u64)(q - 20); break; }
        }
        if (mine != ~0ULL) atomicMin(&s_best, (unsigned long long)mine);
        __syncthreads();
        found = s_best;
        __syncthreads();
        if (found != ~0ULL) break;
    }
    if (threadIdx.x == 0) {
        int ks = (int)found;
        ch[c].ks = ks;
        ch[c].C = shape_const(g + ch[c].seq_off, (u64)ch[c].t_str, ks, (u64)ch[c].t_str);
    }
}
__global__ void __launch_bounds__(256) k_ix_sample(const u8 *g, const ChunkDesc *ch, u32 nch, u64 nsamp, u32 *Xs, u64 *vals) {
    u64 m = (u64)blockIdx.x * blockDim.x + threadIdx.x;
    if (m >= nsamp) return;
    u32 lo = 0, hi = nch - 1;
    while (lo < hi) { u32 mid = (lo + hi + 1) >> 1; if (ch[mid].samp_base <= m) lo = mid; else hi = mid - 1; }
    ChunkDesc c = ch[lo];
    u64 ml = m - c.samp_base;
    u64 j = (u64)c.t_str + 8 + 9 * ml;
    SeedOut o = seed_sample(g + c.seq_off, j, (u64)c.t_str, (u64)c.t_str, c.ks, c.C);
    Xs[m] = o.X | (ml == 0 ? X_FIRST : 0);
    vals[m] = create_cord(c.seq_id, j + ANCHOR_ZERO, o.Y, o.strand);
}
#define REC_TPB 256
#define REC_IPT 4
#define REC_BLK (REC_TPB * REC_IPT)
__device__ __forceinline__ bool ix_is_start(const u32 *Xs, u64 m) {
    u32 x = Xs[m];
    if (x & X_FIRST) return true;
    return (x & X_MASK) != (Xs[m - 1] & X_MASK);
}
__global__ void __launch_bounds__(REC_TPB) k_ix_start_blk(const u32 *Xs, u64 n, u32 *blk_max) {
    __shared__ u32 sh[REC_TPB];
    u64 base = (u64)blockIdx.x * REC_BLK + (u64)threadIdx.x * REC_IPT;
    u32 mx = 0;
    for (int k = 0; k < REC_IPT; k++) { u64 m = base + k; if (m < n && ix_is_start(Xs, m)) mx = (u32)m + 1; }
    sh[threadIdx.x] = mx;
    __syncthreads();
    for (int off = REC_TPB / 2; off > 0; off >>= 1) { if (threadIdx.x < (unsigned)off) sh[threadIdx.x] = max(sh[threadIdx.x], sh[threadIdx.x + off]); __syncthreads(); }
    if (threadIdx.x == 0) blk_max[blockIdx.x] = sh[0];
}
__global__ void __launch_bounds__(1024) k_max_top(u32 *blk, u32 nblk) {
    __shared__ u32 sh[1024];
    __shared__ u32 carry;
    if (threadIdx.x == 0) carry = 0;
    __syncthreads();
    for (u32 base = 0; base < nblk; base += 1024) {
        u32 i = base + threadIdx.x;
        u32 v = i < nblk ? blk[i] : 0;
        sh[threadIdx.x] = v;
        __syncthreads();
        for (int off = 1; off < 1024; off <<= 1) {
            u32 t = threadIdx.x >= (unsigned)off ? sh[threadIdx.x - off] : 0;
            __syncthreads();
            sh[threadIdx.x] = max(sh[threadIdx.x], t);
            __syncthreads();
        }
        u32 c = carry;
        u32 excl = threadIdx.x ? sh[threadIdx.x - 1] : 0;
        if (i < nblk) blk[i] = max(c, excl);
        __syncthreads();
        if (threadIdx.x == 1023) carry = max(c, sh[1023]);
        __syncthreads();
    }
}
__global__ void __launch_bounds__(REC_TPB) k_ix_rec(u32 *Xs, u64 n, const u32 *blk_prefix, i32 *cnt) {
    __shared__ u32 sh[REC_TPB];
    u64 base = (u64)blockIdx.x * REC_BLK + (u64)threadIdx.x * REC_IPT;
    u32 st[REC_IPT];
    u32 mx = 0;
    for (int k = 0; k < REC_IPT; k++) { u64 m = base + k; st[k] = (m < n && ix_is_start(Xs, m)) ? (u32)m + 1 : 0; mx = max(mx, st[k]); }
    sh[threadIdx.x] = mx;
    __syncthreads();
    for (int off = 1; off < REC_TPB; off <<= 1) {
        u32 t = threadIdx.x >= (unsigned)off ? sh[threadIdx.x - off] : 0;
        __syncthreads();
        sh[threadIdx.x] = max(sh[threadIdx.x], t);
        __syncthreads();
    }
    u32 last = max(blk_prefix[blockIdx.x], threadIdx.x ? sh[threadIdx.x - 1] : 0u);
    __syncthreads();
    for (int k = 0; k < REC_IPT; k++) {
        u64 m = base + k;
        if (m >= n) break;
        last = max(last, st[k]);
        if ((((u32)m + 1 - last) & 1) == 0) {
            u32 x = Xs[m];
            Xs[m] = x | X_REC;
            atomicAdd(&cnt[x & X_MASK], 1);
        }
    }
}
__global__ void k_ix_omit(i32 *cnt, u64 n) {
    u64 i = (u64)blockIdx.x * blockDim.x + threadIdx.x;
    if (i < n && cnt[i] > 400) cnt[i] = 0;
}
__global__ void __launch_bounds__(256) k_ix_scatter(const u32 *Xs, const u64 *vals, u64 n, const i32 *dir, i32 *fill, u64 *hs) {
    u64 m = (u64)blockIdx.x * blockDim.x + threadIdx.x;
    if (m >= n) return;
    u32 x = Xs[m];
    if (!(x & X_REC)) return;
    x &= X_MASK;
    i32 b = dir[x], e = dir[x + 1];
    if (e > b) { i32 p = atomicAdd(&fill[x], 1); hs[b + p] = vals[m]; }
}
__global__ void __launch_bounds__(256) k_ix_sort_small(const i32 *dir, u64 nbuckets, u64 *hs, u32 *big, u32 *nbig) {
    u64 b = (u64)blockIdx.x * blockDim.x + threadIdx.x;
    if (b >= nbuckets) return;
    i32 s = dir[b], e = dir[b + 1];
    i32 len = e - s;
    if (len < 2) return;
    if (len > 32) { u32 i = atomicAdd(nbig, 1u); big[i] = (u32)b; return; }
    u64 *a = hs + s;
    for (int i = 1; i < len; i++) {
        u64 v = a[i];
        int j = i - 1;
        while (j >= 0 && a[j] > v) { a[j + 1] = a[j]; j--; }
        a[j + 1] = v;
    }
}
__global__ void __launch_bounds__(64) k_ix_sort_big(const i32 *dir, u64 *hs, const u32 *big, u32 nbig) {
    __shared__ u64 sh[512];
    u32 bi = blockIdx.x;
    if (bi >= nbig) return;
    u32 b = big[bi];
    i32 s = dir[b], len = dir[b + 1] - s;
    for (int i = threadIdx.x; i < 512; i += 64) sh[i] = i < len ? hs[s + i] : ~0ULL;
    __syncthreads();
    for (int k = 2; k <= 512; k <<= 1) {
        for (int j = k >> 1; j > 0; j >>= 1) {
            for (int i = threadIdx.x; i < 512; i += 64) {
                int l = i ^ j;
                if (l > i) {
                    u64 x = sh[i], y = sh[l];
                    bool up = (i & k) == 0;
                    if ((x > y) == up) { sh[i] = y; sh[l] = x; }
                }
            }
            __syncthreads();
        }
    }
    for (int i = threadIdx.x; i < len; i += 64) hs[s + i] = sh[i];
}

__global__ void __launch_bounds__(256) k_f2(const u8 *g, const u64 *seq_off, const u64 *f2_off, u32 nseq, u64 total, F96 *f2) {
    u64 e = (u64)blockIdx.x * blockDim.x + threadIdx.x;
    if (e >= total) return;
    u32 lo = 0, hi = nseq - 1;
    while (lo < hi) { u32 mid = (lo + hi + 1) >> 1; if (f2_off[mid] <= e) lo = mid; else hi = mid - 1; }
    const u8 *s = g + seq_off[lo] + 16 * (e - f2_off[lo]);
    i32 w0 = 0, w1 = 0, w2 = 0;
    u32 prev = s[0];
    for (int j = 1; j <= 48; j++) { u32 cur = s[j]; add2mer(w0, w1, w2, prev, cur); prev = cur; }
    F96 o; o.v0 = w0; o.v1 = w1; o.v2 = w2; o.pad = 0;
    f2[e] = o;
}

__device__ __forceinline__ void prep_fold16(const u32 *x, bool rev, u32 vmask ,
                                            const u32 *vm4 , u32 &codes, u32 &nbits) {
    codes = 0; nbits = 0;
#pragma unroll
    for (int q = 0; q < 4; q++) {
        u32 v = x[q];
        u32 vm = vm4 ? vm4[q] : vmask;
        u32 y = v & 0xFCFCFCFCu;
        u32 n01 = ((((y & 0x7F7F7F7Fu) + 0x7F7F7F7Fu) | y) >> 7) & 0x01010101u;
        u32 t = v & 0x03030303u;
        if (rev) t ^= vm * 3u;
        t &= ~(n01 * 255u);
        u32 c8 = (t | (t >> 6) | (t >> 12) | (t >> 18)) & 0xFFu;
        u32 n4 = (n01 | (n01 >> 7) | (n01 >> 14) | (n01 >> 21)) & 0xFu;
        codes |= c8 << (8 * q); nbits |= n4 << (4 * q);
    }
}
struct PrepGroup { u32 d[4]; u32 cnt; };
__device__ __forceinline__ void prep_group_load(const u8 *rd, u32 L, u32 g, bool rev, bool live, PrepGroup &p) {
    u32 i = 16 * g;
    bool in = live && i < L;
    u32 cnt = in ? (L - i < 16 ? L - i : 16) : 0;
    u32 sh = in ? 16 - cnt : 0;
    u32 a = in ? (rev ? L - 16 - i + sh : i - sh) : 0;
    __builtin_memcpy(p.d, rd + a, 16);
    p.cnt = cnt;
}
__device__ __forceinline__ void prep_group_fold(const PrepGroup &p, bool rev, u32 &codes, u32 &nbits) {
    u32 x[4];
    if (rev) { x[0] = __builtin_bswap32(p.d[3]); x[1] = __builtin_bswap32(p.d[2]); x[2] = __builtin_bswap32(p.d[1]); x[3] = __builtin_bswap32(p.d[0]); }
    else { x[0] = p.d[0]; x[1] = p.d[1]; x[2] = p.d[2]; x[3] = p.d[3]; }
    if (p.cnt == 16) { prep_fold16(x, rev, 0x01010101u, nullptr, codes, nbits); return; }
    codes = 0; nbits = 0;
    if (p.cnt == 0) return;
    u64 lo = x[0] | ((u64)x[1] << 32), hi = x[2] | ((u64)x[3] << 32);
    u32 b = 8 * (16 - p.cnt);
    if (b >= 64) { lo = hi >> (b - 64); hi = 0; } else { lo = (lo >> b) | (hi << (64 - b)); hi >>= b; }
    x[0] = (u32)lo; x[1] = (u32)(lo >> 32); x[2] = (u32)hi; x[3] = (u32)(hi >> 32);
    u32 vm[4];
#pragma unroll
    for (int q = 0; q < 4; q++) {
        u32 c = p.cnt > 4u * q ? p.cnt - 4u * q : 0; c = c > 4 ? 4 : c;
        vm[q] = 0x01010101u & (c == 4 ? 0xFFFFFFFFu : (1u << (8 * c)) - 1u);
        x[q] &= vm[q] * 255u;
    }
    prep_fold16(x, rev, 0, vm, codes, nbits);
}
__device__ __forceinline__ void prep_group_short(const u8 *rd, u32 L, u32 g, bool rev, u32 &codes, u32 &nbits) {
    codes = 0; nbits = 0;
    u32 i = 16 * g;
// ... 2249 lines not shown
```

Before: 2.596 million.

## Batch small host-device copies into one launch and gate lane handover

```diff
diff --git a/linear_amd/build.py b/linear_amd/build.py
--- a/linear_amd/build.py
+++ b/linear_amd/build.py
@@ -30,7 +30,7 @@
 DEVICE_TUS = ["lnr_api.hip", "lnr_gap_kernels.hip", "lnr_output_kernels.hip", "lnr_reader_kernels.hip"]
 OUT_GPU = {"lnr_output_kernels.hip", "lnr_output_hd.h", "lnr_output_hook.h", "lnr_deflate_hd.h", "lnr_inflate_hd.h"}
 RD_GPU = {"lnr_reader_kernels.hip", "lnr_reader_hd.h", "lnr_reader_hook.h", "lnr_inflate_hd.h", "lnr_bam_hd.h"}
-API_HOST = {"lnr_host_util.h", "lnr_ctx.h", "lnr_index.h", "lnr_batch.h", "lnr_gap_stage.h"}
+API_HOST = {"lnr_host_util.h", "lnr_ctx.h", "lnr_handover.h", "lnr_index.h", "lnr_batch.h", "lnr_gap_stage.h"}
 NOT_A_DEP = {"lnr_api.hip": {"lnr_gap_kernels.hip", "lnr_gap_hd.h", "lnr_reader.cpp", "lnr_output.cpp", "linear_filter_main.cpp"} | OUT_GPU | RD_GPU,
              "lnr_gap_kernels.hip": {"lnr_api.hip", "lnr_kernels.hip", "lnr_reader.cpp", "lnr_output.cpp", "linear_filter_main.cpp"} | OUT_GPU | RD_GPU | API_HOST,
              "lnr_output_kernels.hip": set(SOURCES) - OUT_GPU - {"ref_sort.h"},
diff --git a/linear_amd/csrc/lnr_api.hip b/linear_amd/csrc/lnr_api.hip
--- a/linear_amd/csrc/lnr_api.hip
+++ b/linear_amd/csrc/lnr_api.hip
@@ -71,7 +71,7 @@
 std::unique_ptr<Lane> lane_create(lnr_ctx *ctx, int id) {
     std::unique_ptr<Lane> L(new (std::nothrow) Lane());
     if (!L) return nullptr;
-    L->opts = &ctx->opts; L->tun = &ctx->tun; L->ix = &ctx->ix; L->id = id;
+    L->opts = &ctx->opts; L->tun = &ctx->tun; L->ix = &ctx->ix; L->top = ctx; L->id = id;
     if (!L->init(id == 1 ? ctx->tun.lane1_prio : 0)) return nullptr;
     return L;
 }
diff --git a/linear_amd/csrc/lnr_batch.h b/linear_amd/csrc/lnr_batch.h
--- a/linear_amd/csrc/lnr_batch.h
+++ b/linear_amd/csrc/lnr_batch.h
@@ -47,11 +47,13 @@
     S.cap.assign(nj, 0); S.look.assign(nj, 0); S.nanc.assign(nj, 0); S.anc_off.assign(nj, 0);
     if (nj == 0) return f1_reads ? launch_f1(L, f1_reads) : LNR_OK;
     lnr_status s;
-    if ((s = upload_on(L->err, S.j_read, hj.read, st)) != LNR_OK) return s;
-    if ((s = upload_on(L->err, S.j_str, hj.str, st)) != LNR_OK) return s;
-    if ((s = upload_on(L->err, S.j_end, hj.end, st)) != LNR_OK) return s;
-    if ((s = upload_on(L->err, S.j_mode, hj.mode, st)) != LNR_OK) return s;
-    if ((s = upload_on(L->err, S.grp_beg, hj.grp_beg, st)) != LNR_OK) return s;
+    CopyBatch up;
+    if ((s = upload_to(L->err, S.j_read, hj.read, up, st)) != LNR_OK) return s;
+    if ((s = upload_to(L->err, S.j_str, hj.str, up, st)) != LNR_OK) return s;
+    if ((s = upload_to(L->err, S.j_end, hj.end, up, st)) != LNR_OK) return s;
+    if ((s = upload_to(L->err, S.j_mode, hj.mode, up, st)) != LNR_OK) return s;
+    if ((s = upload_to(L->err, S.grp_beg, hj.grp_beg, up, st)) != LNR_OK) return s;
+    LCK(up.flush(st));
     LENSURE(S.j_cap, (size_t)nj * 4);
     LENSURE(S.j_look, (size_t)nj * 4);
     LENSURE(S.j_nanc, (size_t)nj * 4);
@@ -88,6 +90,7 @@
         LCK(rb.add(S.nanc.data(), S.j_nanc.p, (size_t)nj * 4, st));
         LCK(rb.add(S.anc_off.data(), S.j_anc_off.p, (size_t)nj * 8, st));
         LCK(rb.add(&ovf, S.seed_ctl.as<char>() + 16, 4, st));
+        LCK(rb.flush(st));
         LCK(hipStreamSynchronize(st));
         rb.finish();
         if (!ovf) {
@@ -124,7 +127,30 @@
     return LNR_OK;
 }
 
-lnr_status launch_jobs(Lane *L, JobSet &S, const HostJobs &hj) {
+struct HandoverScope : NoCopy {
+    Lane *L; lnr_ctx *c; bool on, held = false;
+    explicit HandoverScope(Lane *l) : L(l), c(l->top) { on = c && c->tun.handover_gate && two_lanes(c) && !c->lane1_off; }
+    void stamp(const char *what) const {
+        if (held && getenv("LNR_DEBUG_TIMES")) fprintf(stderr, "[lnr] handover lane %d %s %.3f\n", L->id, what, std::chrono::duration<double, std::milli>(std::chrono::steady_clock::now().time_since_epoch()).count());
+    }
+    bool enter() {
+        if (!on || held) return false;
+        lnr_ctx *cc = c;
+        bool waited = lnr_ho::handover_enter(c->ho, c->mu, c->cv, L->id, [cc] { return cc->quit; });
+        held = true;
+        stamp(waited ? "gate-passed-after-wait" : "gate-passed");
+        return waited;
+    }
+    void leave() {
+        if (!held) return;
+        stamp("handover-end");
+        held = false;
+        (void)lnr_ho::handover_leave(c->ho, c->mu, c->cv, L->id);
+    }
+    ~HandoverScope() { leave(); }
+};
+
+lnr_status launch_jobs(Lane *L, JobSet &S, const HostJobs &hj, HandoverScope *gate = nullptr) {
     const Index &ix = *L->ix; const Tuning &tun = *L->tun;
     u32 ngrp = (u32)hj.grp_beg.size() - 1;
     if (ngrp == 0) return LNR_OK;
@@ -155,7 +181,8 @@
     Lx.h_order = order;
     laps.lap("order");
     lnr_status s;
-    if ((s = upload_on(L->err, Lx.grp_order, Lx.h_order, sm)) != LNR_OK) return s;
+    CopyBatch up;
+    if ((s = upload_to(L->err, Lx.grp_order, Lx.h_order, up, sm)) != LNR_OK) return s;
     laps.lap("upload-order");
     LENSURE(Lx.j_scr_off, (size_t)nj * 8);
     std::vector<u64> &scr_off = Lx.h_scr_off;
@@ -180,7 +207,8 @@
             void *h = Lx.j_scr_off.host_stage((size_t)nj * 8);
             if (!h) { L->err = "pinned host allocation failed"; return LNR_ERR_NOMEM; }
             memcpy(h, scr_off.data(), (size_t)nj * 8);
-            LCK(words_in(Lx.j_scr_off.p, h, (size_t)nj * 8, sm));
+            LCK(up.add(Lx.j_scr_off.p, h, (u64)nj * 2, sm));
+            LCK(up.flush(sm));
         }
         laps.lap("upload-scr");
         JobArgs A;
@@ -210,6 +238,8 @@
         if (L->tl_round < 4 && g1 <= (1u << 20)) { A.tl = L->tl.as<unsigned long long>() + (size_t)L->tl_round * (1u << 20) * 4; L->tl_n[L->tl_round] = g1; L->tl_nh[L->tl_round] = gm; }
         L->tl_round++;
 #endif
+        bool head_start = gate && g0 == 0 && gate->enter();
+        if (gate && g0 == 0) laps.lap("gate");
         hipStream_t smid = gh > g0 ? L->s_spare : sm;
         bool fork_m = gm > gh && gh > g0, fork_b = g1 > gm && gm > g0;
         if (fork_m || fork_b) LCK(hipEventRecord(L->ev_fork, sm));
@@ -231,10 +261,8 @@
         }
         if (g1 > gm) {
             hipStream_t bulk = fork_b ? sb : sm;
-            if (fork_b) {
-                LCK(hipStreamWaitEvent(sb, L->ev_fork, 0));
-                hipLaunchKernelGGL(k_delay, dim3(1), dim3(64), 0, sb, tun.bulk_delay_ticks); LKCHECK();
-            }
+            if (fork_b) LCK(hipStreamWaitEvent(sb, L->ev_fork, 0));
+            if (fork_b || head_start) { hipLaunchKernelGGL(k_delay, dim3(1), dim3(64), 0, bulk, tun.bulk_delay_ticks); LKCHECK(); }
             JobArgs K = A;
             K.grp_lo = gm; K.grp_hi = g1;
             hipLaunchKernelGGL(k_job, dim3(g1 - gm), dim3(64), lds, bulk, K); LKCHECK();
@@ -259,6 +287,7 @@
         Readback rb;
         if (!rb.begin(L->h_rb[0], ((size_t)n + 1) * 8)) { L->err = "pinned host allocation failed"; return LNR_ERR_NOMEM; }
         LCK(rb.add(B.off.data(), d_off, ((size_t)n + 1) * 8, L->stream));
+        LCK(rb.flush(L->stream));
         LCK(hipStreamSynchronize(L->stream));
         rb.finish();
     }
@@ -279,16 +308,18 @@
         B.gaps_off[i] = go; go += B.gaps_cap[i];
     }
     lnr_status s;
-    if ((s = upload_on(L->err, L->rlen, B.len, L->stream)) != LNR_OK) return s;
-    if ((s = upload_on(L->err, L->pk_off, B.pk_off, L->stream)) != LNR_OK) return s;
+    CopyBatch up;
+    if ((s = upload_to(L->err, L->rlen, B.len, up, L->stream)) != LNR_OK) return s;
+    if ((s = upload_to(L->err, L->pk_off, B.pk_off, up, L->stream)) != LNR_OK) return s;
     LENSURE(L->pk, std::max<u64>(po * 8, 16));
     LENSURE(L->nm, std::max<u64>(po * 4, 16));
-    if ((s = upload_on(L->err, L->nf, B.nf, L->stream)) != LNR_OK) return s;
-    if ((s = upload_on(L->err, L->f1_off, B.f1_off, L->stream)) != LNR_OK) return s;
-    if ((s = upload_on(L->err, L->cords_cap, B.cords_cap, L->stream)) != LNR_OK) return s;
-    if ((s = upload_on(L->err, L->cords_off, B.cords_off, L->stream)) != LNR_OK) return s;
-    if ((s = upload_on(L->err, L->gaps_cap, B.gaps_cap, L->stream)) != LNR_OK) return s;
-    if ((s = upload_on(L->err, L->gaps_off, B.gaps_off, L->stream)) != LNR_OK) return s;
+    if ((s = upload_to(L->err, L->nf, B.nf, up, L->stream)) != LNR_OK) return s;
+    if ((s = upload_to(L->err, L->f1_off, B.f1_off, up, L->stream)) != LNR_OK) return s;
+    if ((s = upload_to(L->err, L->cords_cap, B.cords_cap, up, L->stream)) != LNR_OK) return s;
+    if ((s = upload_to(L->err, L->cords_off, B.cords_off, up, L->stream)) != LNR_OK) return s;
+    if ((s = upload_to(L->err, L->gaps_cap, B.gaps_cap, up, L->stream)) != LNR_OK) return s;
+    if ((s = upload_to(L->err, L->gaps_off, B.gaps_off, up, L->stream)) != LNR_OK) return s;
+    LCK(up.flush(L->stream));
     LENSURE(L->rks, (size_t)n * 4);
     LENSURE(L->f1, std::max<u64>(fo * sizeof(F96), 16));
     LENSURE(L->cords, std::max<u64>(co * 8, 16));
@@ -313,17 +344,16 @@
     return LNR_OK;
 }
 
-lnr_status tail_prepare(Lane *L, const BatchHost &B, TailBuf &tb, const std::vector<u32> *list, hipStream_t st, TailArgs &T) {
+lnr_status counts_out(Lane *L, u32 n, Readback &rb, std::vector<u32> &ncords, hipStream_t st) {
+    ncords.resize(n);
+    if (!rb.begin(L->h_rb[1], (size_t)n * 4)) { L->err = "pinned host allocation failed"; return LNR_ERR_NOMEM; }
+    LCK(rb.add(ncords.data(), L->ncords.p, (size_t)n * 4, st));
+    LCK(rb.flush(st));
+    return LNR_OK;
+}
+
+lnr_status tail_prepare(Lane *L, const BatchHost &B, TailBuf &tb, const std::vector<u32> *list, hipStream_t st, TailArgs &T, const u32 *ncords) {
     u32 n = B.n;
-    std::vector<u32> ncords(n);
-    {
-        Readback rb;
-        PinBuf &pb = L->h_rb[st == L->s_tail ? 2 : 1];
-        if (!rb.begin(pb, (size_t)n * 4)) { L->err = "pinned host allocation failed"; return LNR_ERR_NOMEM; }
-        LCK(rb.add(ncords.data(), L->ncords.p, (size_t)n * 4, st));
-        LCK(hipStreamSynchronize(st));
-        rb.finish();
-    }
     tb.h_off.assign(n, 0); tb.h_cap.assign(n, 0);
     u64 o = 0;
     u32 cnt = list ? (u32)list->size() : n;
@@ -332,15 +362,17 @@
         tb.h_cap[i] = ncords[i] + 4; tb.h_off[i] = o; o += align_up(tail_scratch_bytes(tb.h_cap[i]), 256);
     }
     lnr_status s;
-    if ((s = upload_on(L->err, tb.off, tb.h_off, st)) != LNR_OK) return s;
-    if ((s = upload_on(L->err, tb.cap, tb.h_cap, st)) != LNR_OK) return s;
+    CopyBatch up;
+    if ((s = upload_to(L->err, tb.off, tb.h_off, up, st)) != LNR_OK) return s;
+    if ((s = upload_to(L->err, tb.cap, tb.h_cap, up, st)) != LNR_OK) return s;
     LENSURE(tb.scr, std::max<u64>(o, 16));
     T.read_len = L->rlen.as<u32>(); T.n = cnt; T.list = nullptr;
     if (list) {
         tb.h_list = *list;
-        if ((s = upload_on(L->err, tb.list, tb.h_list, st)) != LNR_OK) return s;
+        if ((s = upload_to(L->err, tb.list, tb.h_list, up, st)) != LNR_OK) return s;
         T.list = tb.list.as<u32>();
     }
+    LCK(up.flush(st));
     T.cords = L->cords.as<u64>(); T.cords_off = L->cords_off.as<u64>(); T.cords_cap = L->cords_cap.as<u32>(); T.ncords = L->ncords.as<u32>();
     T.read_err = L->read_err.as<i32>();
     T.scratch = tb.scr.as<char>(); T.scr_off = tb.off.as<u64>(); T.scr_cap = tb.cap.as<u32>();
@@ -357,31 +389,41 @@
     L->stats.seed_bytes = rb + L->stats.lookups * 8 + L->stats.bucket_entries * 8 + L->stats.anchors * 8;
 }
 
-lnr_status remap_round(Lane *L, const BatchHost &B, HostJobs &j1) {
+lnr_status remap_round(Lane *L, const BatchHost &B, HostJobs &j1, const std::vector<u32> &nc0, std::vector<u32> &nc_a) {
     hipStream_t st = L->stream;
     JobSet &S = L->js[1];
     u32 n = B.n;
     TailArgs T;
     lnr_status s;
-    if ((s = tail_prepare(L, B, L->tb_remap, nullptr, st, T)) != LNR_OK) return s;
+    if ((s = tail_prepare(L, B, L->tb_remap, nullptr, st, T, nc0.data())) != LNR_OK) return s;
     Laps laps;
     laps.lap("tail_prepare");
     LCK(hipMemsetAsync(L->gcursor.p, 0, 4, st));
     hipLaunchKernelGGL(k_tail_a, dim3((T.n + 63) / 64), dim3(64), 0, st, T); LKCHECK();
-    if (!L->h_flags.ensure((size_t)n * 12 + 16)) { L->err = "pinned host allocation failed"; return LNR_ERR_NOMEM; }
-    u32 *remap = L->h_flags.as<u32>(), *ngaps = remap + n, *gpos = ngaps + n, *gtot_p = gpos + n;
-    LCK(copy_words(remap, L->remap.p, n, st));
-    LCK(copy_words(ngaps, L->ngaps.p, n, st));
-    LCK(copy_words(gpos, L->gpos.p, n, st));
-    LCK(copy_words(gtot_p, L->gcursor.p, 1, st));
+    if (!L->h_flags.ensure((size_t)n * 16 + 16)) { L->err = "pinned host allocation failed"; return LNR_ERR_NOMEM; }
+    u32 *remap = L->h_flags.as<u32>(), *ngaps = remap + n, *gpos = ngaps + n, *nca = gpos + n, *gtot_p = nca + n;
+    u64 spec = std::min<u64>(L->tun->gaps_spec ? L->tun->gaps_spec : L->gaps_spec_cap, L->gdense.cap / sizeof(UP));
+    if (!L->h_gaps.ensure(std::max<u64>(spec, 1) * sizeof(UP))) { L->err = "pinned host allocation failed"; return LNR_ERR_NOMEM; }
+    CopyBatch cb;
+    LCK(cb.add(remap, L->remap.p, n, st));
+    LCK(cb.add(ngaps, L->ngaps.p, n, st));
+    LCK(cb.add(gpos, L->gpos.p, n, st));
+    LCK(cb.add(nca, L->ncords.p, n, st));
+    LCK(cb.add(gtot_p, L->gcursor.p, 1, st));
+    LCK(cb.add(L->h_gaps.p, L->gdense.p, spec * sizeof(UP) / 4, st));
+    LCK(cb.flush(st));
     LCK(hipStreamSynchronize(st));
     laps.lap("tail_a+flags");
+    nc_a.assign(nca, nca + n);
     u64 gtot = *gtot_p;
     if (gtot == 0) return LNR_OK;
-    if (!L->h_gaps.ensure(gtot * sizeof(UP))) { L->err = "pinned host allocation failed"; return LNR_ERR_NOMEM; }
+    if (gtot > spec) {
+        if (!L->h_gaps.ensure(gtot * sizeof(UP))) { L->err = "pinned host allocation failed"; return LNR_ERR_NOMEM; }
+        LCK(copy_words(L->h_gaps.p, L->gdense.p, gtot * sizeof(UP) / 4, st));
+        LCK(hipStreamSynchronize(st));
+        L->gaps_spec_cap = gtot + gtot / 2;
+    }
     UP *gaps = L->h_gaps.as<UP>();
-    LCK(copy_words(gaps, L->gdense.p, gtot * sizeof(UP) / 4, st));
-    LCK(hipStreamSynchronize(st));
     for (u32 i = 0; i < n; i++) {
         if (!(remap[i] && ngaps[i])) continue;
         L->stats.remap_reads++;
@@ -406,6 +448,8 @@
     if (!ix.has_index) { L->err = "no index: call lnr_index_build or lnr_index_adopt first"; return LNR_ERR_NO_INDEX; }
     reset_stats(L);
     AllocCount count_(&L->allocs);
+    HandoverScope gate(L);
+    if (attempt == 0) t_copy_launches = 0;
     L->last_n = n; L->last_ncords = 0;
     if (out) { out->n_reads = n; out->n_cords = 0; out->d_cord_off = nullptr; out->d_cords_str = nullptr; out->d_cords_end = nullptr; }
     LENSURE(L->r_off, ((size_t)n + 1) * 8);
@@ -435,11 +479,19 @@
     LCK(hipStreamWaitEvent(L->s_spare, L->ev_start, 0));
     LCK(hipStreamWaitEvent(L->s_bulk, L->ev_start, 0));
     laps.lap("events");
-    if ((s = launch_jobs(L, L->js[0], j0)) != LNR_OK) return s;
+    if ((s = launch_jobs(L, L->js[0], j0, &gate)) != LNR_OK) return s;
+    gate.stamp("round0-enqueued");
     laps.lap("launch0");
-    LCK(hipStreamSynchronize(L->stream));
+    std::vector<u32> nc0, nc_a, nc1;
+    {
+        Readback rb;
+        if ((s = counts_out(L, n, rb, nc0, L->stream)) != LNR_OK) return s;
+        LCK(hipStreamSynchronize(L->stream));
+        rb.finish();
+    }
     HostJobs j1;
-    if ((s = remap_round(L, B, j1)) != LNR_OK) return s;
+    if ((s = remap_round(L, B, j1, nc0, nc_a)) != LNR_OK) return s;
+    gate.leave();
     laps.lap("tailA+seed1+launch1");
     std::vector<u32> late_list, early_list;
     bool early = j1.size() > 0;
@@ -448,16 +500,21 @@
         for (u32 q = 0; q < j1.size(); q++) in_r1[j1.read[q]] = 1;
         for (u32 i = 0; i < n; i++) (in_r1[i] ? late_list : early_list).push_back(i);
         TailArgs TE;
-        if ((s = tail_prepare(L, B, L->tb_early, &early_list, L->s_tail, TE)) != LNR_OK) return s;
+        if ((s = tail_prepare(L, B, L->tb_early, &early_list, L->s_tail, TE, nc_a.data())) != LNR_OK) return s;
         if (TE.n) { hipLaunchKernelGGL(k_tail_b, dim3((TE.n + 63) / 64), dim3(64), 0, L->s_tail, TE); LKCHECK(); }
         LCK(hipEventRecord(L->ev_prep, L->s_tail));
     }
     L->t_job.stop(L->stream);
-    LCK(hipStreamSynchronize(L->stream));
+    {
+        Readback rb;
+        if ((s = counts_out(L, n, rb, nc1, L->stream)) != LNR_OK) return s;
+        LCK(hipStreamSynchronize(L->stream));
+        rb.finish();
+    }
     L->stats.job_ms += L->t_job.ms();
     laps.lap("wait-r1");
     TailArgs T;
-    if ((s = tail_prepare(L, B, L->tb_late, early ? &late_list : nullptr, L->stream, T)) != LNR_OK) return s;
+    if ((s = tail_prepare(L, B, L->tb_late, early ? &late_list : nullptr, L->stream, T, nc1.data())) != LNR_OK) return s;
     L->t_tail.start(L->stream);
     if (T.n) { hipLaunchKernelGGL(k_tail_b, dim3((T.n + 63) / 64), dim3(64), 0, L->stream, T); LKCHECK(); }
     L->t_tail.stop(L->stream);
@@ -478,6 +535,7 @@
         LCK(rb.add(rerr.data(), L->read_err.p, (size_t)n * 4, L->stream));
         if (L->opts->gap_len) LCK(rb.add(&gap_second, L->gap_next.as<u32>() + 16, 4, L->stream));
         if (L->opts->gap_len) LCK(rb.add(&gap_last, L->gap_next.as<u32>() + 24 + 8, 4, L->stream));
+        LCK(rb.flush(L->stream));
         LCK(hipStreamSynchronize(L->stream));
         rb.finish();
     }
@@ -509,14 +567,14 @@
         void *h = L->r_off.host_stage(((size_t)n + 1) * 8);
         if (!h) { L->err = "pinned host allocation failed"; return LNR_ERR_NOMEM; }
         memcpy(h, L->h_cord_off.data(), ((size_t)n + 1) * 8);
-        LCK(words_in(L->r_off.p, h, ((size_t)n + 1) * 8, L->stream));
+        LCK(copy_words(L->r_off.p, h, ((u64)n + 1) * 2, L->stream));
     }
     hipLaunchKernelGGL(k_gather_out, dim3(n), dim3(64), 0, L->stream, L->out_str.as<u64>(), L->out_end.as<u64>(), L->cords_off.as<u64>(), L->nout.as<u32>(),
                        L->r_off.as<u64>(), n, L->r_str.as<u64>(), L->r_end.as<u64>()); LKCHECK();
     L->t_total.stop(L->stream);
     LCK(hipStreamSynchronize(L->stream));
     laps.lap("tailB+gather");
-    if (laps.on) { char b[64]; snprintf(b, sizeof b, " | lane %d allocations so far %u", L->id, L->allocs.load()); laps.out += b; }
+    if (laps.on) { char b[96]; snprintf(b, sizeof b, " | lane %d allocations so far %u, copy launches of this batch %u", L->id, L->allocs.load(), t_copy_launches); laps.out += b; }
     laps.done();
     L->stats.prep_ms = L->t_prep.ms();
     L->stats.total_ms = L->t_total.ms();
diff --git a/linear_amd/csrc/lnr_ctx.h b/linear_amd/csrc/lnr_ctx.h
--- a/linear_amd/csrc/lnr_ctx.h
+++ b/linear_amd/csrc/lnr_ctx.h
@@ -1,4 +1,7 @@
 #pragma once
+#include "lnr_handover.h"
+
+struct lnr_ctx;
 
 namespace {
 
@@ -34,12 +37,16 @@
     u32 nlanes = 2;
     int lane1_prio = 1;
     bool lane1_nomem = false;
+    bool handover_gate = true;
+    u64 gaps_spec = 0;
 };
 
 Tuning tuning_from_env(int device) {
     Tuning t;
     if (const char *e = getenv("LNR_LANES")) { long v = atol(e); if (v == 1 || v == 2) t.nlanes = (u32)v; }
     if (const char *e = getenv("LNR_LANE1_NOMEM")) t.lane1_nomem = atoi(e) != 0;
+    if (const char *e = getenv("LNR_HANDOVER_GATE")) t.handover_gate = atoi(e) != 0;
+    if (const char *e = getenv("LNR_GAPS_SPEC")) { long long v = atoll(e); if (v >= 1) t.gaps_spec = (u64)v; }
     if (const char *e = getenv("LNR_LANE1_PRIO")) { long v = atol(e); if (v >= -1 && v <= 1) t.lane1_prio = (int)v; }
     if (const char *e = getenv("LNR_CAP_SHRINK")) { long v = atol(e); if (v >= 1 && v <= 4096) t.cap_shrink = (u32)v; }
     if (const char *e = getenv("LNR_GAP_TEAMS")) { long v = atol(e); if (v >= 1 && v <= 4096) t.gap_teams = (u32)v; }
@@ -83,6 +90,7 @@
     const lnr_opts *opts = nullptr;
     const Tuning *tun = nullptr;
     const Index *ix = nullptr;
+    struct ::lnr_ctx *top = nullptr;
     int id = 0;
     ErrText err;
     Stream stream, s_spare, s_bulk, s_tail;
@@ -95,10 +103,11 @@
     DevBuf cords, out_str, out_end, cords_off, cords_cap, ncords, nout, read_err;
     DevBuf gaps, gaps_off, gaps_cap, ngaps, remap, gdense, gcursor, gpos;
     PinBuf h_gaps, h_flags;
+    u64 gaps_spec_cap = 0;
     JobSet js[2];
     Launch ln;
     TailBuf tb_remap, tb_early, tb_late;
-    PinBuf h_rb[3];
+    PinBuf h_rb[2];
     DevBuf prof, tl; u32 tl_round = 0, tl_n[4] = {0, 0, 0, 0}; u32 tl_nh[4] = {0, 0, 0, 0};
     DevBuf gap_arena, gap_flag, gap_next, gap_prof, gap_first, gap_list, gap_rank, gap_weight;
     int gap_ext = 0;
@@ -154,6 +163,7 @@
     std::condition_variable cv;
     bool quit = false;
     std::atomic<bool> lane1_off{false};
+    lnr_ho::Handover ho;
     bool lane1_nomem_test = false;
     std::unique_ptr<Lane> lane[2];
 
diff --git a/linear_amd/csrc/lnr_handover.h b/linear_amd/csrc/lnr_handover.h
--- /dev/null
+++ b/linear_amd/csrc/lnr_handover.h
@@ -0,0 +1,30 @@
+#pragma once
+#include <condition_variable>
+#include <mutex>
+
+namespace lnr_ho {
+
+struct Handover {
+    bool in[2] = {false, false};
+};
+
+template <class Quit>
+bool handover_enter(Handover &h, std::mutex &mu, std::condition_variable &cv, int me, Quit quit) {
+    std::unique_lock<std::mutex> lk(mu);
+    bool waited = false;
+    while (h.in[me ^ 1] && !quit()) { waited = true; cv.wait(lk); }
+    h.in[me] = true;
+    return waited;
+}
+
+inline bool handover_leave(Handover &h, std::mutex &mu, std::condition_variable &cv, int me) {
+    {
+        std::lock_guard<std::mutex> g(mu);
+        if (!h.in[me]) return false;
+        h.in[me] = false;
+    }
+    cv.notify_all();
+    return true;
+}
+
+}
diff --git a/linear_amd/csrc/lnr_host_util.h b/linear_amd/csrc/lnr_host_util.h
--- a/linear_amd/csrc/lnr_host_util.h
+++ b/linear_amd/csrc/lnr_host_util.h
@@ -84,10 +84,31 @@
     double ms() { float f = 0; if (hipEventSynchronize(b) != hipSuccess) return 0; (void)hipEventElapsedTime(&f, a, b); return f; }
 };
 
+thread_local unsigned t_copy_launches = 0;
+
+struct CopyBatch {
+    lnr::CopySegs S{};
+    u32 wgs = 0;
+    hipError_t add(void *dst, const void *src, u64 nw, hipStream_t st) {
+        if (!nw) return hipSuccess;
+        if (S.n == COPY_SEGS) { hipError_t e = flush(st); if (e != hipSuccess) return e; }
+        wgs += (u32)std::min<u64>((nw + 63) / 64, 2048);
+        S.s[S.n] = {(const u32 *)src, (u32 *)dst, nw};
+        S.wg_end[S.n++] = wgs;
+        return hipSuccess;
+    }
+    hipError_t flush(hipStream_t st) {
+        if (!S.n) return hipSuccess;
+        hipLaunchKernelGGL(lnr::k_words_out, dim3(wgs), dim3(64), 0, st, S);
+        t_copy_launches++;
+        S.n = 0; wgs = 0;
+        return hipGetLastError();
+    }
+};
 static inline hipError_t copy_words(void *dst, const void *src, u64 nw, hipStream_t st) {
-    if (!nw) return hipSuccess;
-    hipLaunchKernelGGL(lnr::k_words_out, dim3((u32)std::min<u64>((nw + 255) / 256, 1024)), dim3(256), 0, st, (const u32 *)src, (u32 *)dst, nw);
-    return hipGetLastError();
+    CopyBatch cb;
+    (void)cb.add(dst, src, nw, st);
+    return cb.flush(st);
 }
 
 struct Readback {
@@ -95,17 +116,17 @@
     PinBuf *pin = nullptr;
     std::vector<Item> items;
     size_t used = 0;
+    CopyBatch cb;
     bool begin(PinBuf &p, size_t total) { pin = &p; items.clear(); used = 0; return p.ensure(total + 64 * 8); }
     hipError_t add(void *dst, const void *dsrc, size_t bytes, hipStream_t st) {
         size_t o = (used + 15) & ~(size_t)15;
         used = o + bytes;
         items.push_back({dst, o, bytes});
-        return copy_words((char *)pin->p + o, dsrc, bytes / 4, st);
-    }
+        return cb.add((char *)pin->p + o, dsrc, bytes / 4, st);
+    }
+    hipError_t flush(hipStream_t st) { return cb.flush(st); }
     void finish() { for (auto &i : items) if (i.bytes) memcpy(i.dst, (char *)pin->p + i.off, i.bytes); }
 };
-
-static inline hipError_t words_in(void *d_dst, const void *h_pinned, size_t bytes, hipStream_t st) { return copy_words(d_dst, h_pinned, (bytes + 3) / 4, st); }
 
 static const u64 SEQ_PAD = 64;
 static inline u64 align_up(u64 v, u64 a) { return (v + a - 1) / a * a; }
@@ -132,14 +153,22 @@
 #define HIPCK_CTX(c, call) do { hipError_t e__ = (call); if (e__ != hipSuccess) { (c)->err = std::string(#call) + ": " + hipGetErrorString(e__); return LNR_ERR_HIP; } } while (0)
 
 template <class T>
-lnr_status upload_on(ErrText &err, DevBuf &b, const std::vector<T> &v, hipStream_t st) {
+lnr_status upload_to(ErrText &err, DevBuf &b, const std::vector<T> &v, CopyBatch &cb, hipStream_t st) {
     ENSURE_TO(err, b, std::max<size_t>(v.size() * sizeof(T), 16));
     if (!v.empty()) {
         void *h = b.host_stage(v.size() * sizeof(T));
         if (!h) { err = "pinned host allocation failed"; return LNR_ERR_NOMEM; }
         memcpy(h, v.data(), v.size() * sizeof(T));
-        HIPCK_TO(err, words_in(b.p, h, v.size() * sizeof(T), st));
-    }
+        HIPCK_TO(err, cb.add(b.p, h, (v.size() * sizeof(T) + 3) / 4, st));
+    }
+    return LNR_OK;
+}
+template <class T>
+lnr_status upload_on(ErrText &err, DevBuf &b, const std::vector<T> &v, hipStream_t st) {
+    CopyBatch cb;
+    lnr_status s = upload_to(err, b, v, cb, st);
+    if (s != LNR_OK) return s;
+    HIPCK_TO(err, cb.flush(st));
     return LNR_OK;
 }
 
diff --git a/linear_amd/csrc/lnr_kernels.hip b/linear_amd/csrc/lnr_kernels.hip
--- a/linear_amd/csrc/lnr_kernels.hip
+++ b/linear_amd/csrc/lnr_kernels.hip
@@ -8,8 +8,15 @@
 #include "lnr_wave.h"
 namespace lnr {
 
-__global__ void __launch_bounds__(256) k_words_out(const u32 *src, u32 *dst, u64 n) {
-    for (u64 i = (u64)blockIdx.x * blockDim.x + threadIdx.x; i < n; i += (u64)gridDim.x * blockDim.x) dst[i] = src[i];
+#define COPY_SEGS 8
+struct CopySeg { const u32 *src; u32 *dst; u64 words; };
+struct CopySegs { CopySeg s[COPY_SEGS]; u32 wg_end[COPY_SEGS]; u32 n; };
+__global__ void __launch_bounds__(64) k_words_out(CopySegs S) {
+    u32 b = blockIdx.x, k = 0;
+    while (k + 1 < S.n && b >= S.wg_end[k]) k++;
+    u32 w0 = k ? S.wg_end[k - 1] : 0, nwg = S.wg_end[k] - w0;
+    const u32 *src = S.s[k].src; u32 *dst = S.s[k].dst; u64 n = S.s[k].words;
+    for (u64 i = (u64)(b - w0) * 64 + threadIdx.x; i < n; i += (u64)nwg * 64) dst[i] = src[i];
 }
 
 #if defined(K_JOB_WAVES) && K_JOB_WAVES > 4
```

Result: faster. 2.799 million, median of 6 (+7.8%).
